# pachyderm-io/pfs

Hardware: AMD Instinct MI355X
Metric: GiB/s device-resident CDC rolling-hash + chunk content-hash (higher is better)
Workload: dtype u8

## Files before the change

### include/pfscdc.h

```cpp
#ifndef PFSCDC_H
#define PFSCDC_H

#include <stddef.h>
#include <stdint.h>

#ifdef __cplusplus
extern "C" {
#endif

#define PFSCDC_OK 0
#define PFSCDC_EINVAL -1
#define PFSCDC_EHIP -2
#define PFSCDC_ENOMEM -3
#define PFSCDC_EUNSUPPORTED -4
#define PFSCDC_ESTATE -5
#define PFSCDC_ECALLBACK -6
#define PFSCDC_ECORRUPT -7
#define PFSCDC_ENOTFOUND -8

typedef struct pfscdc_params {
  uint32_t average_bits;
  uint32_t reserved;
  int64_t seed;
  int64_t min_chunk;
// ... 43 lines not shown
int pfscdc_wait(pfscdc_ctx* ctx);

uint64_t pfscdc_num_segments(const pfscdc_ctx* ctx);
const pfscdc_segment* pfscdc_segments(const pfscdc_ctx* ctx);
const uint64_t* pfscdc_file_segment_begin(const pfscdc_ctx* ctx);

#define PFSCDC_OPT_REF_IDS 1u
#define PFSCDC_OPT_CUTS_ONLY 2u
#define PFSCDC_OPT_CTEXT_IN_PLACE 4u
int pfscdc_set_options(pfscdc_ctx* ctx, uint32_t options);
const pfscdc_ref* pfscdc_refs(const pfscdc_ctx* ctx);
int pfscdc_last_ref_ms(pfscdc_ctx* ctx, float* ms);

int pfscdc_get_chunks(pfscdc_ctx* ctx, const void* ctext, uint64_t nbytes, int ctext_on_device,
                      const uint64_t* chunk_offsets, uint32_t nchunks, const pfscdc_ref* refs,
                      void* ptext, int ptext_on_device, uint8_t* ok);
int pfscdc_last_get_ms(pfscdc_ctx* ctx, float* ms);

typedef struct pfscdc_slice {
  uint32_t chunk;
  uint32_t reserved;
  uint64_t offset;
  uint64_t size;
} pfscdc_slice;

int pfscdc_read_slices(pfscdc_ctx* ctx, const void* ctext, uint64_t nbytes, int ctext_on_device,
                       const uint64_t* chunk_offsets, uint32_t nchunks, const pfscdc_ref* refs,
                       const uint8_t* verified, const pfscdc_slice* slices, uint32_t nslices,
                       void* out, int out_on_device, uint8_t* chunk_ok, uint8_t* slice_ok);
int pfscdc_last_read_timings(pfscdc_ctx* ctx, float out[2]);

#define PFSCDC_TAR_USTAR 1
#define PFSCDC_TAR_PAX 2
typedef struct pfscdc_tar_file {
  const char* path;
  uint32_t first;
  uint32_t count;
} pfscdc_tar_file;

int pfscdc_tar_header(const char* path, uint64_t size, uint8_t out[512]);
int pfscdc_tar_layout(const pfscdc_tar_file* files, uint32_t nfiles, const uint64_t* sizes,
                      uint64_t* entry_offsets, uint64_t* total);
int pfscdc_tar_head(const char* path, uint64_t size, int format, uint8_t* out, uint64_t cap,
                    uint64_t* len);
int pfscdc_tar_layout_format(const pfscdc_tar_file* files, uint32_t nfiles, const uint64_t* sizes,
                             int format, uint64_t* entry_offsets, uint64_t* total);
int pfscdc_set_tar_format(pfscdc_ctx* ctx, int format);
int pfscdc_read_tar(pfscdc_ctx* ctx, const void* ctext, uint64_t nbytes, int ctext_on_device,
                    const uint64_t* chunk_offsets, uint32_t nchunks, const pfscdc_ref* refs,
                    const uint8_t* verified, const pfscdc_tar_file* files, uint32_t nfiles,
                    const pfscdc_slice* slices, uint32_t nslices, uint64_t begin, uint64_t len,
                    void* out, int out_on_device, uint8_t* chunk_ok, uint64_t* nwritten);
int pfscdc_last_frame_ms(pfscdc_ctx* ctx, float* ms);

int pfscdc_create_refs(pfscdc_ctx* ctx, const void* bytes, uint64_t nbytes, int bytes_on_device,
                       const uint64_t* chunk_offsets, uint32_t nchunks, uint8_t* content_hashes,
                       const uint8_t* hash_known, pfscdc_ref* refs);
int pfscdc_commit_refs(pfscdc_ctx* ctx, const void* bytes, uint64_t nbytes, int bytes_on_device,
                       const uint64_t* chunk_offsets, uint32_t nchunks, uint8_t* content_hashes,
                       const uint8_t* hash_known, pfscdc_ref* refs, uint8_t* segment_hashes);
int pfscdc_hash_data_refs(pfscdc_ctx* ctx, const uint8_t* hashes, uint32_t n, uint8_t out[32]);
int pfscdc_last_create_ms(pfscdc_ctx* ctx, float* ms);
int pfscdc_last_create_timings(pfscdc_ctx* ctx, float out[2]);
int pfscdc_last_create_form(pfscdc_ctx* ctx, int* split);


int pfscdc_candidates(pfscdc_ctx* ctx, const void* bytes, uint64_t nbytes, int bytes_on_device,
                      uint64_t halo, uint64_t* out, uint64_t cap, uint64_t* n);

int pfscdc_hash_ranges(pfscdc_ctx* ctx, const void* bytes, uint64_t nbytes, int bytes_on_device,
                       const uint64_t* begins, const uint64_t* sizes, uint32_t n, uint8_t* out);

uint64_t pfscdc_debug_candidates(pfscdc_ctx* ctx, uint64_t* out, uint64_t cap);

uint64_t pfscdc_debug_hash_queue(pfscdc_ctx* ctx, uint32_t* order, uint64_t order_cap,
                                 uint32_t* next, uint64_t next_cap, uint64_t* bin_bytes);
uint64_t pfscdc_debug_scan_plan(pfscdc_ctx* ctx, uint32_t* slots, uint64_t cap);

int pfscdc_last_scan_bytes(pfscdc_ctx* ctx, uint64_t* out);

int pfscdc_last_timings(pfscdc_ctx* ctx, float out[5]);
int pfscdc_last_kernel_spans(pfscdc_ctx* ctx, float out[2]);
int pfscdc_last_kernel_clocks(pfscdc_ctx* ctx, float out[2]);

void* pfscdc_host_alloc(uint64_t nbytes);
void pfscdc_host_free(void* p);

int pfscdc_fill_synthetic(pfscdc_ctx* ctx, void* dev_bytes, const uint64_t* file_offsets,
                          uint32_t nfiles, uint64_t seed);

#define PFSCDC_SYNTH_RANDOM 0u
#define PFSCDC_SYNTH_DEDUP_BLOCKS 1u
#define PFSCDC_SYNTH_DEDUP_FILES 2u
int pfscdc_fill_synthetic_ex(pfscdc_ctx* ctx, void* dev_bytes, const uint64_t* file_offsets,
                             uint32_t nfiles, uint64_t seed, uint32_t mode);
int pfscdc_fill_synthetic_pieces(pfscdc_ctx* ctx, void* dev_bytes, const uint64_t* piece_offsets,
                                 uint32_t npieces, const uint32_t* file_ids,
                                 const uint64_t* file_starts, uint64_t seed, uint32_t mode);


typedef struct pfscdc_dataref {
  uint8_t hash[32];
  int64_t offset_bytes;
  int64_t size_bytes;
} pfscdc_dataref;

typedef struct pfscdc_chunk_ref {
  uint64_t chunk_index;
  int64_t size_bytes;
  int32_t edge;
  int32_t has_ref;
  pfscdc_ref ref;
  int32_t copied;
  int32_t reserved2;
} pfscdc_chunk_ref;

typedef struct pfscdc_annotation_out {
  uint64_t user;
  int32_t has_data_ref;
  int32_t reserved;
  pfscdc_dataref data_ref;
} pfscdc_annotation_out;

typedef int (*pfscdc_writer_cb)(void* user, const pfscdc_chunk_ref* chunk,
                                const pfscdc_annotation_out* annotations, uint32_t n);

typedef struct pfscdc_writer pfscdc_writer;

typedef struct pfscdc_full_dataref {
  pfscdc_ref ref;
  int64_t ref_size;
  int32_t edge;
  int32_t reserved;
  pfscdc_dataref data;
} pfscdc_full_dataref;

typedef struct pfscdc_store pfscdc_store;
int pfscdc_store_create(pfscdc_store** out);
int pfscdc_store_destroy(pfscdc_store* s);
int pfscdc_store_put(pfscdc_store* s, const uint8_t id[32], const void* ctext, uint64_t n);
int pfscdc_store_get(const pfscdc_store* s, const uint8_t id[32], const void** ctext,
                     uint64_t* n);
uint64_t pfscdc_store_count(const pfscdc_store* s);
int pfscdc_store_read(pfscdc_ctx* ctx, const pfscdc_store* s, const pfscdc_full_dataref* drs,
                      uint32_t n, void* out, uint64_t out_cap, int out_on_device,
                      uint64_t* nwritten);
int pfscdc_store_read_tar(pfscdc_ctx* ctx, const pfscdc_store* s, const pfscdc_tar_file* files,
                          uint32_t nfiles, const pfscdc_full_dataref* drs, uint32_t ndrs,
                          uint64_t begin, uint64_t len, void* out, uint64_t out_cap,
                          int out_on_device, uint64_t* nwritten);

int pfscdc_writer_create(pfscdc_ctx* ctx, pfscdc_writer_cb cb, void* user,
                         uint64_t batch_bytes, pfscdc_writer** out);
int pfscdc_writer_annotate(pfscdc_writer* w, uint64_t user);
int pfscdc_writer_write(pfscdc_writer* w, const void* data, uint64_t n);
int pfscdc_writer_close(pfscdc_writer* w);
int64_t pfscdc_writer_chunk_count(const pfscdc_writer* w);
int64_t pfscdc_writer_annotation_count(const pfscdc_writer* w);
int pfscdc_writer_destroy(pfscdc_writer* w);

int pfscdc_writer_set_store(pfscdc_writer* w, pfscdc_store* store, int upload);
int pfscdc_writer_copy(pfscdc_writer* w, const pfscdc_full_dataref* dr);
int pfscdc_writer_prefetch(pfscdc_writer* w, const pfscdc_full_dataref* drs, uint32_t n);
int pfscdc_merge_file_hash(pfscdc_ctx* ctx, pfscdc_store* store, const pfscdc_full_dataref* drs,
                           uint32_t n, uint8_t out[32]);

// ... 267 lines not shown
```

### pfs_amd/_lib.py

```python
from __future__ import annotations

import ctypes as C
import os
import threading

_HERE = os.path.dirname(os.path.abspath(__file__))
LIB_PATH = os.environ.get("PFSCDC_LIB") or os.path.join(_HERE, "libpfscdc.so")

PFSCDC_OK = 0
PFSCDC_EINVAL = -1
PFSCDC_EHIP = -2
PFSCDC_ENOMEM = -3
PFSCDC_EUNSUPPORTED = -4
PFSCDC_ESTATE = -5
PFSCDC_ECALLBACK = -6
PFSCDC_ECORRUPT = -7
PFSCDC_ENOTFOUND = -8
TAR_USTAR, TAR_PAX = 1, 2

SEG_VALID = 1
SEG_CUT = 2
OPT_REF_IDS = 1
OPT_CUTS_ONLY = 2
OPT_CTEXT_IN_PLACE = 4
SCAN_SKIPPED_FIRST_MIN = 1
SCAN_SKIPPED_CUTS = 2

EXPORTED = [
    "pfscdc_default_params", "pfscdc_table", "pfscdc_go_int63", "pfscdc_ctx_create",
    "pfscdc_ctx_destroy", "pfscdc_last_error", "pfscdc_set_stream", "pfscdc_stream_wait",
    "pfscdc_stream_handle",
    "pfscdc_scan",
    "pfscdc_scan_async", "pfscdc_wait", "pfscdc_num_segments", "pfscdc_segments",
    "pfscdc_file_segment_begin", "pfscdc_debug_candidates", "pfscdc_debug_hash_queue",
    "pfscdc_debug_scan_plan", "pfscdc_last_timings",
    "pfscdc_last_scan_bytes", "pfscdc_commit_refs",
    "pfscdc_set_options", "pfscdc_refs", "pfscdc_last_ref_ms", "pfscdc_get_chunks",
    "pfscdc_last_get_ms",
    "pfscdc_host_alloc", "pfscdc_host_free", "pfscdc_fill_synthetic", "pfscdc_fill_synthetic_ex", "pfscdc_writer_create",
    "pfscdc_writer_annotate", "pfscdc_writer_write", "pfscdc_writer_close",
    "pfscdc_writer_chunk_count", "pfscdc_writer_annotation_count", "pfscdc_writer_destroy",
    "pfscdc_create_refs", "pfscdc_last_create_ms", "pfscdc_form_chunks",
    "pfscdc_uw_create", "pfscdc_uw_put", "pfscdc_uw_delete", "pfscdc_uw_close",
    "pfscdc_uw_num_filesets", "pfscdc_uw_fileset", "pfscdc_uw_destroy", "pfscdc_uw_last_error", "pfscdc_uw_timings",
    "pfscdc_uw_trim_cache", "pfscdc_uw_cached_arena_bytes",
    "pfscdc_path_clean",
    "pfscdc_hash_data_refs", "pfscdc_store_create", "pfscdc_store_destroy", "pfscdc_store_put",
    "pfscdc_store_get", "pfscdc_store_count", "pfscdc_writer_set_store", "pfscdc_writer_copy",
    "pfscdc_merge_file_hash", "pfscdc_last_create_timings", "pfscdc_last_create_form", "pfscdc_writer_prefetch",
    "pfscdc_candidates", "pfscdc_hash_ranges", "pfscdc_fill_synthetic_pieces",
    "pfscdc_last_kernel_spans", "pfscdc_last_kernel_clocks", "pfscdc_order_hash_after",
    "pfscdc_set_knob", "pfscdc_get_knob", "pfscdc_knob_info", "pfscdc_last_scan_mode",
    "pfscdc_deal", "pfscdc_group_create", "pfscdc_group_destroy", "pfscdc_group_size",
    "pfscdc_group_ctx", "pfscdc_group_last_error", "pfscdc_group_scan",
    "pfscdc_group_scan_resident", "pfscdc_group_num_segments", "pfscdc_group_segments",
    "pfscdc_group_file_segment_begin", "pfscdc_group_refs", "pfscdc_group_part_begin",
    "pfscdc_group_index_device", "pfscdc_group_last_timings", "pfscdc_uw_create_group",
    "pfscdc_group_scan_stream",
    "pfscdc_read_slices", "pfscdc_last_read_timings", "pfscdc_store_read",
    "pfscdc_tar_header", "pfscdc_tar_layout", "pfscdc_read_tar", "pfscdc_last_frame_ms",
    "pfscdc_store_read_tar", "pfscdc_tar_head", "pfscdc_tar_layout_format", "pfscdc_set_tar_format",
    "pfscdc_uw_set_store", "pfscdc_index_list_count", "pfscdc_index_list_entries",
    "pfscdc_index_list_blob", "pfscdc_index_list_datarefs", "pfscdc_index_list_tar_files",
    "pfscdc_index_list_free", "pfscdc_index_decode_host", "pfscdc_index_filter_list",
    "pfscdc_index_read", "pfscdc_last_index_stats", "pfscdc_last_index_timings",
    "pfscdc_index_merge", "pfscdc_index_merge_deletive", "pfscdc_index_merge_ctx",
    "pfscdc_last_merge_stats", "pfscdc_last_merge_timings", "pfscdc_shard",
    "pfscdc_fsw_create", "pfscdc_fsw_delete", "pfscdc_fsw_copy", "pfscdc_fsw_copy_lists",
    "pfscdc_fsw_copy_filesets", "pfscdc_fsw_close", "pfscdc_fsw_fileset",
    "pfscdc_fsw_last_error", "pfscdc_fsw_destroy",
    "pfscdc_dev_list_upload", "pfscdc_dev_list_download", "pfscdc_dev_list_count",
    "pfscdc_dev_list_num_datarefs", "pfscdc_dev_list_blob_len", "pfscdc_dev_list_free",
    "pfscdc_index_read_dev", "pfscdc_index_merge_dev", "pfscdc_dev_list_tar_layout",
    "pfscdc_dev_list_read_tar", "pfscdc_last_resident_stats",
    "pfscdc_source_host", "pfscdc_source_host_error", "pfscdc_file_infos_free",
    "pfscdc_source_open", "pfscdc_source_open_list", "pfscdc_source_list", "pfscdc_source_count",
    "pfscdc_source_infos", "pfscdc_source_free", "pfscdc_last_source_stats",
    "pfscdc_last_source_timings",
    "pfscdc_glob_match", "pfscdc_glob_literal_prefix", "pfscdc_debug_glob_program",
    "pfscdc_debug_glob_masks", "pfscdc_debug_list_scan",
    "pfscdc_diff_host", "pfscdc_diff_pairs_free", "pfscdc_source_diff", "pfscdc_diff_count",
    "pfscdc_diff_pairs", "pfscdc_diff_side", "pfscdc_diff_free", "pfscdc_last_diff_stats",
    "pfscdc_last_diff_timings",
    "pfscdc_copy_map_host", "pfscdc_dev_list_copy_map", "pfscdc_copy_map_list",
    "pfscdc_last_copy_map_stats", "pfscdc_last_copy_map_timings", "pfscdc_uw_copy",
    "pfscdc_uw_copy_file",
]


class Params(C.Structure):
    _fields_ = [("average_bits", C.c_uint32), ("reserved", C.c_uint32), ("seed", C.c_int64),
                ("min_chunk", C.c_int64), ("max_chunk", C.c_int64)]


class Segment(C.Structure):
    _fields_ = [("offset", C.c_uint64), ("size", C.c_uint64), ("file", C.c_uint32),
                ("flags", C.c_uint32), ("hash", C.c_uint8 * 32)]


class DataRef(C.Structure):
    _fields_ = [("hash", C.c_uint8 * 32), ("offset_bytes", C.c_int64), ("size_bytes", C.c_int64)]


class RefC(C.Structure):
    _fields_ = [("id", C.c_uint8 * 32), ("dek", C.c_uint8 * 32)]


class ChunkRef(C.Structure):
    _fields_ = [("chunk_index", C.c_uint64), ("size_bytes", C.c_int64), ("edge", C.c_int32),
                ("has_ref", C.c_int32), ("ref", RefC), ("copied", C.c_int32),
                ("reserved2", C.c_int32)]


class FullDataRef(C.Structure):
    _fields_ = [("ref", RefC), ("ref_size", C.c_int64), ("edge", C.c_int32),
                ("reserved", C.c_int32), ("data", DataRef)]


class TarFile(C.Structure):
    _fields_ = [("path", C.c_char_p), ("first", C.c_uint32), ("count", C.c_uint32)]


def tar_files(files):
    arr = (TarFile * max(1, len(files)))()
    for i, (path, first, count) in enumerate(files):
        p = path.encode() if isinstance(path, str) else bytes(path)
        if b"\0" in p:
            raise ValueError(f"tar entry {path!r}: NUL in the name")
        arr[i] = TarFile(p, first, count)
    return arr


class IndexFilter(C.Structure):
    _fields_ = [("lower", C.c_char_p), ("upper", C.c_char_p), ("prefix", C.c_char_p),
# ... 60 lines not shown


def slice_dtype():
    global SLICE_DTYPE
    if SLICE_DTYPE is None:
        import numpy as np
        SLICE_DTYPE = np.dtype([("chunk", "<u4"), ("reserved", "<u4"), ("offset", "<u8"),
                                ("size", "<u8")])
        assert SLICE_DTYPE.itemsize == 24
    return SLICE_DTYPE


def ref_dtype():
    global REF_DTYPE
    if REF_DTYPE is None:
        import numpy as np
        REF_DTYPE = np.dtype([("id", "u1", (32,)), ("dek", "u1", (32,))])
        assert REF_DTYPE.itemsize == 64
    return REF_DTYPE


def segment_dtype():
    global SEGMENT_DTYPE
    if SEGMENT_DTYPE is None:
        import numpy as np
        SEGMENT_DTYPE = np.dtype([("offset", "<u8"), ("size", "<u8"), ("file", "<u4"),
                                  ("flags", "<u4"), ("hash", "u1", (32,))])
        assert SEGMENT_DTYPE.itemsize == 56
    return SEGMENT_DTYPE


_lib = None
_lock = threading.Lock()


class PfsCdcError(RuntimeError):
    def __init__(self, code: int, msg: str):
        super().__init__(f"pfscdc error {code}: {msg}")
        self.code = code


def load() -> C.CDLL:
    global _lib
    with _lock:
        if _lib is not None:
            return _lib
        if not os.path.exists(LIB_PATH):
            raise ImportError(f"{LIB_PATH} is missing: build it with `make` or "
                              "`python -c 'import __graft_entry__ as g; g.build()'`")
        try:
            import torch
        except ImportError:
            pass
        lib = C.CDLL(LIB_PATH)
        u64, i64, u32, i32, vp = C.c_uint64, C.c_int64, C.c_uint32, C.c_int, C.c_void_p
        P = C.POINTER
        sig = {
            "pfscdc_default_params": (None, [P(Params)]),
            "pfscdc_table": (i32, [i64, P(u64)]),
            "pfscdc_go_int63": (i32, [i64, P(i64), i32]),
            "pfscdc_ctx_create": (i32, [P(Params), i32, P(vp)]),
            "pfscdc_ctx_destroy": (i32, [vp]),
            "pfscdc_last_error": (C.c_char_p, [vp]),
            "pfscdc_set_stream": (i32, [vp, vp]),
            "pfscdc_stream_wait": (i32, [vp, vp]),
            "pfscdc_stream_handle": (vp, [vp]),
            "pfscdc_order_hash_after": (i32, [vp, vp]),
            "pfscdc_scan": (i32, [vp, vp, u64, i32, P(u64), u32]),
            "pfscdc_scan_async": (i32, [vp, vp, u64, i32, P(u64), u32]),
            "pfscdc_wait": (i32, [vp]),
            "pfscdc_num_segments": (u64, [vp]),
            "pfscdc_segments": (P(Segment), [vp]),
            "pfscdc_file_segment_begin": (P(u64), [vp]),
            "pfscdc_debug_candidates": (u64, [vp, P(u64), u64]),
            "pfscdc_debug_hash_queue": (u64, [vp, vp, u64, vp, u64, P(u64)]),
            "pfscdc_debug_scan_plan": (u64, [vp, vp, u64]),
            "pfscdc_last_timings": (i32, [vp, P(C.c_float)]),
            "pfscdc_last_scan_bytes": (i32, [vp, P(u64)]),
            "pfscdc_last_scan_mode": (i32, [vp, P(u32)]),
            "pfscdc_set_knob": (i32, [C.c_char_p, i64]),
            "pfscdc_get_knob": (i32, [C.c_char_p, P(i64)]),
            "pfscdc_knob_info": (C.c_char_p, [i32, P(i64), P(i64), P(i64)]),
            "pfscdc_last_kernel_spans": (i32, [vp, P(C.c_float)]),
            "pfscdc_last_kernel_clocks": (i32, [vp, P(C.c_float)]),
            "pfscdc_set_options": (i32, [vp, u32]),
            "pfscdc_refs": (vp, [vp]),
            "pfscdc_last_ref_ms": (i32, [vp, P(C.c_float)]),
            "pfscdc_get_chunks": (i32, [vp, vp, u64, i32, P(u64), u32, vp, vp, i32, vp]),
            "pfscdc_last_get_ms": (i32, [vp, P(C.c_float)]),
            "pfscdc_host_alloc": (vp, [u64]),
            "pfscdc_host_free": (None, [vp]),
            "pfscdc_fill_synthetic": (i32, [vp, vp, P(u64), u32, u64]),
            "pfscdc_fill_synthetic_ex": (i32, [vp, vp, P(u64), u32, u64, u32]),
            "pfscdc_writer_create": (i32, [vp, WRITER_CB, vp, u64, P(vp)]),
            "pfscdc_writer_annotate": (i32, [vp, u64]),
            "pfscdc_writer_write": (i32, [vp, vp, u64]),
            "pfscdc_writer_close": (i32, [vp]),
            "pfscdc_writer_chunk_count": (i64, [vp]),
            "pfscdc_writer_annotation_count": (i64, [vp]),
            "pfscdc_writer_destroy": (i32, [vp]),
            "pfscdc_create_refs": (i32, [vp, vp, u64, i32, P(u64), u32, vp, vp, vp]),
            "pfscdc_commit_refs": (i32, [vp, vp, u64, i32, P(u64), u32, vp, vp, vp, vp]),
            "pfscdc_last_create_ms": (i32, [vp, P(C.c_float)]),
            "pfscdc_last_create_timings": (i32, [vp, P(C.c_float)]),
            "pfscdc_last_create_form": (i32, [vp, P(i32)]),
            "pfscdc_form_chunks": (i32, [vp, P(C.c_uint32), u32, P(u64), vp, vp, u64, P(u64)]),
            "pfscdc_uw_create": (i32, [vp, i64, P(Params), UW_CB, vp, P(vp)]),
            "pfscdc_uw_put": (i32, [vp, C.c_char_p, C.c_char_p, i32, vp, u64]),
            "pfscdc_uw_delete": (i32, [vp, C.c_char_p, C.c_char_p]),
            "pfscdc_uw_close": (i32, [vp]),
            "pfscdc_uw_num_filesets": (u32, [vp]),
            "pfscdc_uw_fileset": (i32, [vp, u32, P(FilesetInfo)]),
            "pfscdc_uw_destroy": (i32, [vp]),
            "pfscdc_uw_last_error": (C.c_char_p, [vp]),
            "pfscdc_uw_timings": (i32, [vp, P(C.c_double)]),
            "pfscdc_uw_trim_cache": (i32, [i32, P(u64), P(u32)]),
            "pfscdc_uw_cached_arena_bytes": (u64, []),
            "pfscdc_path_clean": (i32, [C.c_char_p, i32, C.c_char_p, u64]),
            "pfscdc_hash_data_refs": (i32, [vp, vp, u32, vp]),
            "pfscdc_store_create": (i32, [P(vp)]),
            "pfscdc_store_destroy": (i32, [vp]),
            "pfscdc_store_put": (i32, [vp, vp, vp, u64]),
            "pfscdc_store_get": (i32, [vp, vp, P(vp), P(u64)]),
            "pfscdc_store_count": (u64, [vp]),
            "pfscdc_writer_set_store": (i32, [vp, vp, i32]),
            "pfscdc_writer_copy": (i32, [vp, P(FullDataRef)]),
            "pfscdc_writer_prefetch": (i32, [vp, P(FullDataRef), u32]),
            "pfscdc_merge_file_hash": (i32, [vp, vp, P(FullDataRef), u32, vp]),
            "pfscdc_candidates": (i32, [vp, vp, u64, i32, u64, P(u64), u64, P(u64)]),
            "pfscdc_hash_ranges": (i32, [vp, vp, u64, i32, P(u64), P(u64), u32, vp]),
            "pfscdc_fill_synthetic_pieces": (i32, [vp, vp, P(u64), u32, P(C.c_uint32), P(u64),
                                                   u64, u32]),
            "pfscdc_deal": (i32, [P(u64), u32, u32, P(C.c_uint32)]),
            "pfscdc_group_create": (i32, [P(Params), P(C.c_int), u32, u32, P(vp)]),
            "pfscdc_group_destroy": (i32, [vp]),
            "pfscdc_group_size": (u32, [vp]),
            "pfscdc_group_ctx": (vp, [vp, u32]),
            "pfscdc_group_last_error": (C.c_char_p, [vp]),
            "pfscdc_group_scan": (i32, [vp, vp, u64, P(u64), u32]),
            "pfscdc_group_scan_resident": (i32, [vp, P(vp), P(u64), u32, P(C.c_uint32)]),
            "pfscdc_group_num_segments": (u64, [vp]),
            "pfscdc_group_segments": (vp, [vp]),
            "pfscdc_group_file_segment_begin": (P(u64), [vp]),
            "pfscdc_group_refs": (vp, [vp]),
            "pfscdc_group_part_begin": (P(C.c_uint32), [vp]),
            "pfscdc_group_index_device": (i32, [vp, P(vp), P(vp), P(C.c_int)]),
            "pfscdc_group_last_timings": (i32, [vp, P(C.c_float), P(C.c_float), P(u64)]),
            "pfscdc_uw_create_group": (i32, [vp, i64, P(Params), UW_CB, vp, P(vp)]),
            "pfscdc_group_scan_stream": (i32, [vp, vp, u64]),
            "pfscdc_read_slices": (i32, [vp, vp, u64, i32, P(u64), u32, vp, vp, vp, u32, vp, i32,
                                         vp, vp]),
            "pfscdc_last_read_timings": (i32, [vp, P(C.c_float)]),
            "pfscdc_store_read": (i32, [vp, vp, P(FullDataRef), u32, vp, u64, i32, P(u64)]),
            "pfscdc_tar_header": (i32, [C.c_char_p, u64, vp]),
            "pfscdc_tar_layout": (i32, [P(TarFile), u32, P(u64), P(u64), P(u64)]),
            "pfscdc_tar_head": (i32, [C.c_char_p, u64, i32, vp, u64, P(u64)]),
            "pfscdc_tar_layout_format": (i32, [P(TarFile), u32, P(u64), i32, P(u64), P(u64)]),
            "pfscdc_set_tar_format": (i32, [vp, i32]),
            "pfscdc_read_tar": (i32, [vp, vp, u64, i32, P(u64), u32, vp, vp, P(TarFile), u32, vp,
                                      u32, u64, u64, vp, i32, vp, P(u64)]),
            "pfscdc_last_frame_ms": (i32, [vp, P(C.c_float)]),
            "pfscdc_store_read_tar": (i32, [vp, vp, P(TarFile), u32, P(FullDataRef), u32, u64,
                                            u64, vp, u64, i32, P(u64)]),
            "pfscdc_uw_set_store": (i32, [vp, vp]),
            "pfscdc_index_list_count": (u32, [vp]),
            "pfscdc_index_list_entries": (P(IndexEntry), [vp]),
# ... 156 lines not shown
```

### pfs_amd/cdc.py

```python
from __future__ import annotations

import ctypes as C
from dataclasses import dataclass
from typing import Optional, Sequence

import numpy as np

from . import _lib


SYNTH_RANDOM, SYNTH_DEDUP_BLOCKS, SYNTH_DEDUP_FILES = 0, 1, 2


@dataclass(frozen=True)
class ChunkParams:
    average_bits: int = 23
    seed: int = 1
    min_chunk: int = 1_000_000
    max_chunk: int = 20_000_000

    def to_c(self) -> _lib.Params:
        return _lib.Params(self.average_bits, 0, self.seed, self.min_chunk, self.max_chunk)


# ... 63 lines not shown
            pass

    def _check(self, rc: int, what: str) -> None:
        if rc:
            msg = self.lib.pfscdc_last_error(self.ctx)
            raise _lib.PfsCdcError(rc, f"{what}: {msg.decode() if msg else ''}")

    def set_stream(self, stream_handle: Optional[int]) -> None:
        self._check(self.lib.pfscdc_set_stream(self.ctx, stream_handle or None), "set_stream")

    def order_hash_after(self, other: Optional["Chunker"]) -> None:
        self._check(self.lib.pfscdc_order_hash_after(self.ctx, other.ctx if other else None),
                    "order_hash_after")

    def wait_for(self, other: "Chunker") -> None:
        h = self.lib.pfscdc_stream_handle(other.ctx)
        self._check(self.lib.pfscdc_stream_wait(self.ctx, h), "stream_wait")

    def _after_torch(self, *tensors) -> None:
        for t in tensors:
            if t is not None and getattr(t, "is_cuda", False):
                import torch

                h = torch.cuda.current_stream(t.device).cuda_stream
                self._check(self.lib.pfscdc_stream_wait(self.ctx, h or None), "stream_wait")
                return

    def scan_async(self, data, file_offsets: Sequence[int]) -> None:
        offs = _offsets_array(file_offsets)
        self._offs_keep = offs
        nfiles = len(offs) - 1
        on_dev = 0
        if hasattr(data, "is_cuda") and data.is_cuda:
            if data.dtype.itemsize != 1 or not data.is_contiguous():
                raise ValueError("device data must be a contiguous uint8 tensor")
            ptr, nbytes, on_dev = data.data_ptr(), data.numel(), 1
            self._data_keep = data
            self._after_torch(data)
        else:
            arr = np.frombuffer(data, dtype=np.uint8) if isinstance(data, (bytes, bytearray, memoryview)) \
                else np.ascontiguousarray(data, dtype=np.uint8)
            self._data_keep = arr
            ptr, nbytes = (arr.ctypes.data if arr.size else None), arr.size
        rc = self.lib.pfscdc_scan_async(self.ctx, ptr, nbytes, on_dev,
                                        offs.ctypes.data_as(C.POINTER(C.c_uint64)), nfiles)
        self._check(rc, "scan_async")
        self._nfiles = nfiles

    def wait(self) -> ScanResult:
        self._check(self.lib.pfscdc_wait(self.ctx), "wait")
        n = self.lib.pfscdc_num_segments(self.ctx)
        dt = _lib.segment_dtype()
        if n:
            ptr = self.lib.pfscdc_segments(self.ctx)
            buf = C.string_at(ptr, n * dt.itemsize)
            segs = np.frombuffer(buf, dtype=dt).copy()
        else:
            segs = np.zeros(0, dtype=dt)
        bp = self.lib.pfscdc_file_segment_begin(self.ctx)
        begin = np.ctypeslib.as_array(bp, shape=(self._nfiles + 1,)).copy() if bp else \
            np.zeros(self._nfiles + 1, dtype=np.uint64)
        refs = None
        if self.ref_ids:
            rdt = _lib.ref_dtype()
            rp = self.lib.pfscdc_refs(self.ctx)
            refs = np.frombuffer(C.string_at(rp, n * rdt.itemsize), dtype=rdt).copy() \
                if (n and rp) else np.zeros(0, dtype=rdt)
        return ScanResult(segs, begin, refs=refs)

    def scan(self, data, file_offsets: Sequence[int]) -> ScanResult:
        self.scan_async(data, file_offsets)
        return self.wait()

    def timings(self) -> dict:
        out = (C.c_float * 5)()
        self._check(self.lib.pfscdc_last_timings(self.ctx, out), "timings")
        t = dict(zip(["scan", "compact", "select", "hash", "total"], list(out)))
        sp = (C.c_float * 2)()
        self._check(self.lib.pfscdc_last_kernel_spans(self.ctx, sp), "kernel_spans")
        t["scan_span"], t["hash_span"] = sp[0], sp[1]
        ck = (C.c_float * 2)()
        self._check(self.lib.pfscdc_last_kernel_clocks(self.ctx, ck), "kernel_clocks")
        t["scan_mhz"], t["hash_mhz"] = ck[0], ck[1]
        if self.ref_ids:
            ms = C.c_float()
            self._check(self.lib.pfscdc_last_ref_ms(self.ctx, C.byref(ms)), "timings")
            t["ref_ids"] = ms.value
        return t

    def get_chunks(self, ctext, chunk_offsets: Sequence[int], refs: np.ndarray, out=None):
        offs = _offsets_array(chunk_offsets)
        n = len(offs) - 1
        refs = np.ascontiguousarray(refs, dtype=_lib.ref_dtype())
        if len(refs) != n:
            raise ValueError("one ref per chunk")
        self._after_torch(ctext, out)
        if hasattr(ctext, "is_cuda") and ctext.is_cuda:
            cptr, nbytes, con = ctext.data_ptr(), ctext.numel(), 1
        else:
            arr = np.ascontiguousarray(np.frombuffer(ctext, dtype=np.uint8)
                                       if isinstance(ctext, (bytes, bytearray)) else ctext,
                                       dtype=np.uint8)
            cptr, nbytes, con = (arr.ctypes.data if arr.size else None), arr.size, 0
            self._get_keep = arr
        if out is not None:
            optr, oon, res = out.data_ptr(), 1, out
        else:
            res = np.empty(nbytes, dtype=np.uint8)
            optr, oon = (res.ctypes.data if nbytes else None), 0
        ok = np.zeros(max(n, 1), dtype=np.uint8)
        rc = self.lib.pfscdc_get_chunks(self.ctx, cptr, nbytes, con,
                                        offs.ctypes.data_as(C.POINTER(C.c_uint64)), n,
                                        refs.ctypes.data if n else None, optr, oon,
                                        ok.ctypes.data)
        self._check(rc, "get_chunks")
        return res, ok[:n].astype(bool)


    @staticmethod
    def _stored_batch(chunk_offsets, refs, slices, verified):
        offs = _offsets_array(chunk_offsets)
        n = len(offs) - 1
        refs = np.ascontiguousarray(refs, dtype=_lib.ref_dtype())
        if len(refs) != n:
            raise ValueError("one ref per chunk")
        sdt = _lib.slice_dtype()
        if isinstance(slices, np.ndarray) and slices.dtype == sdt:
            sl = np.ascontiguousarray(slices)
        else:
            sl = np.zeros(len(slices), dtype=sdt)
            for i, (ch, o, z) in enumerate(slices):
                sl[i] = (ch, 0, o, z)
        ver = None
        if verified is not None:
            ver = np.ascontiguousarray(np.asarray(verified).astype(np.uint8))
            if len(ver) != n:
                raise ValueError("one verified mark per chunk")
        return offs, n, refs, sl, len(sl), ver

    def _ctext_arg(self, ctext):
        if hasattr(ctext, "is_cuda") and ctext.is_cuda:
            if ctext.dtype.itemsize != 1 or not ctext.is_contiguous():
                raise ValueError("device ctext must be a contiguous uint8 tensor")
            return ctext.data_ptr(), ctext.numel(), 1
        arr = np.ascontiguousarray(np.frombuffer(ctext, dtype=np.uint8)
                                   if isinstance(ctext, (bytes, bytearray)) else ctext,
                                   dtype=np.uint8)
        self._get_keep = arr
        return (arr.ctypes.data if arr.size else None), arr.size, 0

    @staticmethod
    def _out_arg(out, need: int, what: str):
        if out is None:
            res = np.empty(need, dtype=np.uint8)
            return res, (res.ctypes.data if need else None), 0
        if isinstance(out, np.ndarray):
            if out.dtype != np.uint8 or not out.flags.c_contiguous or out.size < need:
                raise ValueError(f"out must be a contiguous uint8 array of {what}")
            return out, (out.ctypes.data if out.size else None), 0
        if out.dtype.itemsize != 1 or not out.is_contiguous() or out.numel() < need:
            raise ValueError(f"out must be a contiguous uint8 tensor of {what}")
        return out, (out.data_ptr() if out.numel() else None), int(out.is_cuda)

    def read_slices(self, ctext, chunk_offsets: Sequence[int], refs: np.ndarray, slices,
                    out=None, verified=None):
        offs, n, refs, sl, ns, ver = self._stored_batch(chunk_offsets, refs, slices, verified)
# ... 317 lines not shown
```

### pfs_amd/csrc/cdc_kernels.hip

```cpp
#include <hip/hip_runtime.h>
#include <stdint.h>
#include <stdlib.h>

#include <algorithm>
#include <type_traits>

#include "pfscdc_internal.h"

#define PFS_DEV __device__ __forceinline__

namespace pfscdc {


PFS_DEV uint64_t rotl1_64(uint64_t x) { return (x << 1) | (x >> 63); }

PFS_DEV uint32_t tab_addr(uint32_t w, uint32_t lane_off, int j) {
  return __builtin_amdgcn_perm(w, lane_off, 0x0c0c0000u | ((4u + (uint32_t)j) << 8));
}

template <typename T>
PFS_DEV T lds_load(const uint8_t* lds, uint32_t byte_addr) {
  return *reinterpret_cast<const T*>(lds + byte_addr);
}

// ... 589 lines not shown
  __syncthreads();
  if (threadIdx.x == 0) {
    __threadfence();
    *s_flag = atomicAdd(done_ctr, 1u) == gridDim.x - 1 ? 1u : 0u;
  }
  __syncthreads();
  const bool last = *s_flag != 0;
  if (last) __threadfence();
  return last;
}

template <int BLOCK>
PFS_DEV void compact_tiles(const TileRec* __restrict__ recs, uint64_t ntiles, uint64_t n,
                           uint64_t* __restrict__ entries, uint64_t* __restrict__ n_entries,
                           uint64_t* s_wave) {
  uint64_t carry = 0;
  for (uint64_t base = 0; base < ntiles; base += BLOCK) {
    const uint64_t t = base + threadIdx.x;
    uint32_t c = 0;
    uint64_t e = 0;
    if (t < ntiles) {
      c = recs[t].count;
      e = c <= (uint32_t)kTileK ? c : 1;
    }
    uint64_t total;
    const uint64_t ex = block_exscan<BLOCK>(e, s_wave, &total) + carry;
    if (t < ntiles) {
      const uint64_t ts = t * kTile;
      if (c <= (uint32_t)kTileK) {
        uint32_t o[kTileK];
#pragma unroll
        for (int i = 0; i < kTileK; i++) o[i] = i < (int)c ? recs[t].off[i] : ~0u;
#pragma unroll
        for (int i = 0; i < kTileK; i++) {
          uint32_t rank = 0;
#pragma unroll
          for (int j = 0; j < kTileK; j++) rank += o[j] < o[i];
          if (i < (int)c) entries[ex + rank] = ts + o[i];
        }
      } else {
        const uint64_t te = (ts + kTile < n) ? ts + kTile : n;
        entries[ex] = kDenseBit | (te - 1);
      }
    }
    carry += total;
  }
  if (threadIdx.x == 0) *n_entries = carry;
}

template <int BLOCK>
PFS_DEV uint64_t segcompact_block(const pfscdc_segment* __restrict__ slots,
                                  const uint64_t* __restrict__ seg_base,
                                  const uint64_t* __restrict__ nseg, uint32_t nfiles,
                                  pfscdc_segment* __restrict__ segs,
                                  uint64_t* __restrict__ seg_begin, uint64_t* s_wave) {
  uint64_t carry = 0;
  for (uint64_t base = 0; base < nfiles; base += BLOCK) {
    const uint64_t f = base + threadIdx.x;
    const uint64_t c = f < nfiles ? nseg[f] : 0;
    uint64_t total;
    const uint64_t ex = block_exscan<BLOCK>(c, s_wave, &total) + carry;
    if (f < nfiles) {
      seg_begin[f] = ex;
      const pfscdc_segment* src = slots + seg_base[f];
      for (uint64_t i = 0; i < c; i++) segs[ex + i] = src[i];
    }
    carry += total;
  }
  if (threadIdx.x == 0) seg_begin[nfiles] = carry;
  return carry;
}

PFS_DEV uint32_t lpt_key(uint64_t size) {
  const uint64_t nblk = (size + 127) / 128;
  const uint64_t k = nblk >> 6;
  return 1023u - (uint32_t)(k < 1023 ? k : 1023);
}

template <int BLOCK>
PFS_DEV void lpt_order_block(const pfscdc_segment* __restrict__ segs, uint64_t n,
                             uint32_t* __restrict__ order, uint32_t* __restrict__ counter,
                             uint32_t* hist, uint64_t* s_wave,
                             const uint64_t* __restrict__ offs = nullptr, uint64_t bin_bytes = 0,
                             uint32_t* __restrict__ next = nullptr, uint64_t* qlen = nullptr) {
  const bool bins = next && offs && bin_bytes;
  auto binned = [&](uint64_t i) {
    const uint32_t f = segs[i].file;
    return bins && offs[f + 1] - offs[f] <= bin_bytes;
  };
  auto entry = [&](uint64_t i, uint32_t& key) {
    if (binned(i)) {
      const uint32_t f = segs[i].file;
      key = lpt_key(offs[f + 1] - offs[f]);
      return i == 0 || segs[i - 1].file != f;
    }
    key = lpt_key(segs[i].size);
    return true;
  };
  constexpr int kPer = 1024 / BLOCK;
  static_assert(1024 % BLOCK == 0, "bins split evenly over the block");
  for (int b = 0; b < kPer; b++) hist[threadIdx.x * kPer + b] = 0;
  __syncthreads();
  for (uint64_t i = threadIdx.x; i < n; i += BLOCK) {
    uint32_t key;
    if (entry(i, key)) atomicAdd(&hist[key], 1u);
    if (bins) next[i] = binned(i) && i + 1 < n && segs[i + 1].file == segs[i].file
                            ? (uint32_t)(i + 1) : kNoNext;
  }
  __syncthreads();
  uint32_t local[kPer];
  uint64_t sum = 0;
  for (int b = 0; b < kPer; b++) {
    local[b] = hist[threadIdx.x * kPer + b];
    sum += local[b];
  }
  uint64_t total;
  uint64_t start = block_exscan<BLOCK>(sum, s_wave, &total);
  for (int b = 0; b < kPer; b++) {
    hist[threadIdx.x * kPer + b] = (uint32_t)start;
    start += local[b];
  }
  __syncthreads();
  for (uint64_t i = threadIdx.x; i < n; i += BLOCK) {
    uint32_t key;
    if (entry(i, key)) order[atomicAdd(&hist[key], 1u)] = (uint32_t)i;
  }
  if (threadIdx.x == 0) {
    *counter = 0;
    if (qlen) *qlen = total;
  }
}


PFS_DEV uint64_t rescan_first(const uint8_t* __restrict__ data, const uint64_t* __restrict__ T,
                              uint64_t a, uint64_t b, uint64_t mask) {
  const uint32_t lane = threadIdx.x & 63u;
  constexpr uint64_t W = 256;
  for (uint64_t base = a; base <= b; base += 64 * W) {
    const uint64_t st = base + lane * W;
    const uint64_t en = (st + W - 1 < b) ? st + W - 1 : b;
    uint64_t found = kNone;
    if (st <= en) {
      uint64_t h = 0;
      for (int k = 0; k < 64; k++) h = rotl1_64(h) ^ T[data[st - 63 + k]];
      if ((h & mask) == 0) found = st;
      for (uint64_t i = st + 1; found == kNone && i <= en; i++) {
        h = rotl1_64(h) ^ T[data[i - 64]] ^ T[data[i]];
        if ((h & mask) == 0) found = i;
      }
    }
    found = wave_min_u64(found);
    if (found != kNone) return found;
  }
  return kNone;
}

PFS_DEV void select_file(
    const uint8_t* __restrict__ data, const uint64_t* __restrict__ T,
    const uint64_t* __restrict__ entries, const uint64_t* __restrict__ n_entries,
    const uint64_t* __restrict__ offs, const uint64_t* __restrict__ seg_base, uint64_t f,
    uint64_t mask, uint64_t min_chunk, uint64_t max_chunk,
    pfscdc_segment* __restrict__ slots, uint64_t* __restrict__ nseg) {
  const uint32_t lane = threadIdx.x & 63u;
  const uint64_t fs = offs[f], fe = offs[f + 1];
  const uint64_t sb = seg_base[f], cap = seg_base[f + 1] - sb;
  const uint64_t ne = *n_entries;
  pfscdc_segment* out = slots + sb;
  uint64_t count = 0;
  auto emit = [&](uint64_t s, uint64_t size, uint32_t flags) {
    if (lane == 0 && count < cap) {
      out[count].offset = s - fs;
      out[count].size = size;
      out[count].file = (uint32_t)f;
      out[count].flags = flags;
    }
    count++;
  };
  uint64_t k = 0;
  {
    const uint64_t key = fs + min_chunk - 1;
    uint64_t lo = 0, hi = ne;
    while (hi - lo > 64) {
      const uint64_t step = (hi - lo + 63) / 64;
      const uint64_t i = lo + lane * step;
      const bool below = i < hi && (entries[i] & ~kDenseBit) < key;
      const uint32_t cnt = (uint32_t)__popcll(__ballot(below));
      if (cnt == 0) {
        hi = lo;
      } else {
        const uint64_t top = lo + (uint64_t)cnt * step;
        lo = lo + (uint64_t)(cnt - 1) * step + 1;
        hi = top < hi ? top : hi;
      }
    }
    const uint64_t i = lo + lane;
    const bool below = i < hi && (entries[i] & ~kDenseBit) < key;
    k = lo + (uint64_t)__popcll(__ballot(below));
  }
  uint64_t s = fs;
  while (true) {
    const uint64_t lo = s + min_chunk - 1;
    if (lo >= fe) break;
    const uint64_t hi = s + max_chunk - 1;
    const uint64_t limit = hi < fe - 1 ? hi : fe - 1;
    while (k < ne && (entries[k] & ~kDenseBit) < lo) k++;
    uint64_t c = kNone;
    for (uint64_t kk = k; kk < ne; kk++) {
      const uint64_t e = entries[kk];
      const uint64_t v = e & ~kDenseBit;
      if (!(e & kDenseBit)) {
        if (v <= limit) c = v;
        break;
      }
      const uint64_t ts = (v / kTile) * kTile;
      const uint64_t a = lo > ts ? lo : ts;
      const uint64_t bnd = v < limit ? v : limit;
      if (a <= bnd) {
        c = rescan_first(data, T, a, bnd, mask);
        if (c != kNone) break;
      }
      if (v >= limit) break;
    }
    uint64_t cut;
    if (c != kNone) cut = c;
    else if (hi <= fe - 1) cut = hi;
    else break;
    emit(s, cut + 1 - s, PFSCDC_SEG_VALID | PFSCDC_SEG_CUT);
    s = cut + 1;
  }
  if (s < fe) emit(s, fe - s, PFSCDC_SEG_VALID);
  if (lane == 0) {
    for (uint64_t i = count; i < cap; i++) out[i].flags = 0;
    nseg[f] = count;
  }
}

__global__ __launch_bounds__(kSelectBlock) void select_kernel(
    const uint8_t* __restrict__ data, const uint64_t* __restrict__ T,
    const uint64_t* __restrict__ entries, const uint64_t* __restrict__ n_entries,
    const uint64_t* __restrict__ offs, const uint64_t* __restrict__ seg_base, uint32_t nfiles,
    uint64_t mask, uint64_t min_chunk, uint64_t max_chunk,
    pfscdc_segment* __restrict__ slots, uint64_t* __restrict__ nseg, uint32_t* done_ctr,
    pfscdc_segment* __restrict__ segs, uint64_t* __restrict__ seg_begin,
    uint32_t* __restrict__ order, uint32_t* __restrict__ counter, uint64_t bin_bytes,
    uint32_t* __restrict__ next, uint64_t* __restrict__ qlen) {
  __shared__ uint32_t hist[1024];
  __shared__ uint64_t s_wave[kSelectBlock / 64 + 1];
  __shared__ uint32_t s_flag;
  const uint64_t f = ((uint64_t)blockIdx.x * kSelectBlock + threadIdx.x) >> 6;
  if (f < nfiles)
    select_file(data, T, entries, n_entries, offs, seg_base, f, mask, min_chunk, max_chunk,
                slots, nseg);
  if (!last_block_done(done_ctr, &s_flag)) return;
  const uint64_t total = segcompact_block<kSelectBlock>(slots, seg_base, nseg, nfiles, segs,
                                                        seg_begin, s_wave);
  __threadfence_block();
  __syncthreads();
  if (order)
    lpt_order_block<kSelectBlock>(segs, total, order, counter, hist, s_wave, offs, bin_bytes,
                                  next, qlen);
}


__global__ __launch_bounds__(kCompactBlock) void hash_order_kernel(
    const pfscdc_segment* __restrict__ segs, const uint64_t* __restrict__ seg_count,
    uint32_t* __restrict__ order, uint32_t* __restrict__ counter) {
  __shared__ uint32_t hist[1024];
  __shared__ uint64_t s_wave[kCompactBlock / 64 + 1];
  lpt_order_block<kCompactBlock>(segs, *seg_count, order, counter, hist, s_wave);
}


constexpr uint64_t kB2IV[8] = {
    0x6a09e667f3bcc908ULL, 0xbb67ae8584caa73bULL, 0x3c6ef372fe94f82bULL,
    0xa54ff53a5f1d36f1ULL, 0x510e527fade682d1ULL, 0x9b05688c2b3e6c1fULL,
    0x1f83d9abfb41bd6bULL, 0x5be0cd19137e2179ULL};

template <typename T>
PFS_DEV T pick4(uint32_t j, T v0, T v1, T v2, T v3) {
  return j == 0 ? v0 : j == 1 ? v1 : j == 2 ? v2 : v3;
}

constexpr uint32_t kSigmaPack[12][4] = {
#define PK(a, b, c, d) ((uint32_t)(a) * 8u | (uint32_t)(b) * 8u << 8 | (uint32_t)(c) * 8u << 16 | (uint32_t)(d) * 8u << 24)
#define ROW(s0, s1, s2, s3, s4, s5, s6, s7, s8, s9, s10, s11, s12, s13, s14, s15) \
  {PK(s0, s1, s14, s15), PK(s2, s3, s8, s9), PK(s4, s5, s10, s11), PK(s6, s7, s12, s13)}
    ROW(0, 1, 2, 3, 4, 5, 6, 7, 8, 9, 10, 11, 12, 13, 14, 15),
    ROW(14, 10, 4, 8, 9, 15, 13, 6, 1, 12, 0, 2, 11, 7, 5, 3),
    ROW(11, 8, 12, 0, 5, 2, 15, 13, 10, 14, 3, 6, 7, 1, 9, 4),
    ROW(7, 9, 3, 1, 13, 12, 11, 14, 2, 6, 5, 10, 4, 0, 15, 8),
    ROW(9, 0, 5, 7, 2, 4, 10, 15, 14, 1, 11, 12, 6, 8, 3, 13),
    ROW(2, 12, 6, 10, 0, 11, 8, 3, 4, 13, 7, 5, 15, 14, 1, 9),
    ROW(12, 5, 1, 15, 14, 13, 4, 10, 0, 7, 6, 3, 9, 2, 8, 11),
    ROW(13, 11, 7, 14, 12, 1, 3, 9, 5, 0, 15, 4, 8, 6, 2, 10),
    ROW(6, 15, 14, 9, 11, 3, 0, 8, 12, 2, 13, 7, 1, 4, 10, 5),
    ROW(10, 2, 8, 4, 7, 6, 1, 5, 15, 11, 9, 14, 3, 12, 13, 0),
    ROW(0, 1, 2, 3, 4, 5, 6, 7, 8, 9, 10, 11, 12, 13, 14, 15),
    ROW(14, 10, 4, 8, 9, 15, 13, 6, 1, 12, 0, 2, 11, 7, 5, 3),
#undef ROW
#undef PK
};

PFS_DEV uint64_t mk64(uint32_t lo, uint32_t hi) { return ((uint64_t)hi << 32) | lo; }
PFS_DEV uint64_t xor_rotr32(uint64_t x, uint64_t y) {
  return mk64((uint32_t)(x >> 32) ^ (uint32_t)(y >> 32), (uint32_t)x ^ (uint32_t)y);
}
template <int N>
PFS_DEV uint64_t xor_rotr(uint64_t x, uint64_t y) {
  const uint32_t lo = (uint32_t)x ^ (uint32_t)y, hi = (uint32_t)(x >> 32) ^ (uint32_t)(y >> 32);
  return mk64(__builtin_amdgcn_alignbit(hi, lo, N), __builtin_amdgcn_alignbit(lo, hi, N));
}
PFS_DEV uint64_t xor_rotr63(uint64_t x, uint64_t y) {
  const uint32_t lo = (uint32_t)x ^ (uint32_t)y, hi = (uint32_t)(x >> 32) ^ (uint32_t)(y >> 32);
  return mk64(__builtin_amdgcn_alignbit(lo, hi, 31), __builtin_amdgcn_alignbit(hi, lo, 31));
}

template <int CTRL>
PFS_DEV uint64_t quad_perm64(uint64_t x) {
  const uint32_t lo = (uint32_t)__builtin_amdgcn_mov_dpp((int)(uint32_t)x, CTRL, 0xF, 0xF, true);
  const uint32_t hi = (uint32_t)__builtin_amdgcn_mov_dpp((int)(uint32_t)(x >> 32), CTRL, 0xF, 0xF, true);
  return mk64(lo, hi);
}

#define PFS_G(a, b, c, d, x, y)  \
  do {                           \
    a = a + b + (x);             \
    d = xor_rotr32(d, a);        \
    c = c + d;                   \
    b = xor_rotr<24>(b, c);      \
    a = a + b + (y);             \
    d = xor_rotr<16>(d, a);      \
    c = c + d;                   \
    b = xor_rotr63(b, c);        \
  } while (0)

PFS_DEV void msg_load_full(uint4& m0, uint4& m1, const uint8_t* p) {
  __builtin_memcpy(&m0, p, 16);
  __builtin_memcpy(&m1, p + 16, 16);
}

PFS_DEV uint32_t keep_bytes(int64_t k) {
  return k >= 4 ? 0xffffffffu : k <= 0 ? 0u : (1u << (8 * (uint32_t)k)) - 1u;
}
// ... 136 lines not shown
  "v_lshl_add_u64 v[100:101], v[100:101], 0, v[102:103]\n"             \
  "v_xor_b32 v110, v108, v100\n"                                       \
  "v_xor_b32 v111, v109, v101\n"                                       \
  "v_alignbit_b32 v106, v111, v110, 16\n"                              \
  "v_alignbit_b32 v107, v110, v111, 16\n"                              \
  "v_lshl_add_u64 v[104:105], v[104:105], 0, v[106:107]\n"             \
  "v_xor_b32 v110, v102, v104\n"                                       \
  "v_xor_b32 v111, v103, v105\n"                                       \
  "v_alignbit_b32 v102, v110, v111, 31\n"                              \
  "v_alignbit_b32 v103, v111, v110, 31\n"
#define PFS_G_ASM_FIRST(X, Y)                                          \
  "v_lshl_add_u64 v[100:101], %[a0], 0, " X "\n"                      \
  "v_lshl_add_u64 v[100:101], v[100:101], 0, %[b0]\n"                 \
  "v_bitop3_b32 v108, %[d0h], %[dth], v101 bitop3:0x96\n"             \
  "v_bitop3_b32 v109, %[d0l], %[dtl], v100 bitop3:0x96\n"             \
  "v_lshl_add_u64 v[104:105], %[c0], 0, v[108:109]\n"                 \
  "v_xor_b32 v110, %[b0l], v104\n"                                    \
  "v_xor_b32 v111, %[b0h], v105\n"                                    \
  "v_alignbit_b32 v102, v111, v110, 24\n"                             \
  "v_alignbit_b32 v103, v110, v111, 24\n"                             \
  "v_lshl_add_u64 v[100:101], v[100:101], 0, " Y "\n"                 \
  "v_lshl_add_u64 v[100:101], v[100:101], 0, v[102:103]\n"            \
  "v_xor_b32 v110, v108, v100\n"                                      \
  "v_xor_b32 v111, v109, v101\n"                                      \
  "v_alignbit_b32 v106, v111, v110, 16\n"                             \
  "v_alignbit_b32 v107, v110, v111, 16\n"                             \
  "v_lshl_add_u64 v[104:105], v[104:105], 0, v[106:107]\n"            \
  "v_xor_b32 v110, v102, v104\n"                                      \
  "v_xor_b32 v111, v103, v105\n"                                      \
  "v_alignbit_b32 v102, v110, v111, 31\n"                             \
  "v_alignbit_b32 v103, v111, v110, 31\n"
#define PFS_QP_ID "[0,1,2,3]"
#define PFS_QP_R1 "[1,2,3,0]"
#define PFS_QP_R2 "[2,3,0,1]"
#define PFS_QP_R3 "[3,0,1,2]"
#define PFS_DIAG_G PFS_G_ASM(PFS_QP_R3, PFS_QP_R1, PFS_QP_R2, "%[x2l]", "%[x2h]", "%[x3]")
#define PFS_ROUND_OPS(x0_, x1_, x2_, x3_)                                                \
  : "+{v[100:101]}"(a), "+{v[102:103]}"(b), "+{v[104:105]}"(c), "+{v[106:107]}"(d)      \
  : [x0] "v"(x0_), [x0l] "v"((uint32_t)(x0_)), [x0h] "v"((uint32_t)((x0_) >> 32)),      \
    [x1] "v"(x1_), [x2l] "v"((uint32_t)(x2_)), [x2h] "v"((uint32_t)((x2_) >> 32)),       \
    [x3] "v"(x3_)                                                                        \
  : "vcc", "v108", "v109", "v110", "v111"
#define PFS_ROUND_FIRST(a0_, b0_, c0_, d0_, dt_, x0_, x1_, x2_, x3_)                          \
  asm volatile(PFS_G_ASM_FIRST("%[x0]", "%[x1]") PFS_DIAG_G                                    \
               : "=&{v[100:101]}"(a), "=&{v[102:103]}"(b), "=&{v[104:105]}"(c),                  \
                 "=&{v[106:107]}"(d)                                                           \
               : [a0] "v"(a0_), [b0] "v"(b0_), [b0l] "v"((uint32_t)(b0_)),                     \
                 [b0h] "v"((uint32_t)((b0_) >> 32)), [c0] "v"(c0_),                            \
                 [d0l] "v"((uint32_t)(d0_)), [d0h] "v"((uint32_t)((d0_) >> 32)),               \
                 [dtl] "v"((uint32_t)(dt_)), [dth] "v"((uint32_t)((dt_) >> 32)),               \
                 [x0] "v"(x0_), [x1] "v"(x1_), [x2l] "v"((uint32_t)(x2_)),                      \
                 [x2h] "v"((uint32_t)((x2_) >> 32)), [x3] "v"(x3_)                              \
               : "vcc", "v108", "v109", "v110", "v111")
#define PFS_ROUND(FIRST, x0_, x1_, x2_, x3_)                                                  \
  do {                                                                                        \
    if (FIRST)                                                                                \
      asm volatile(PFS_G_ASM_PLAIN("%[x0]", "%[x1]") PFS_DIAG_G                    \
                 PFS_ROUND_OPS(x0_, x1_, x2_, x3_));                                          \
    else                                                                                      \
      asm volatile(PFS_G_ASM(PFS_QP_R1, PFS_QP_R3, PFS_QP_R2, "%[x0l]", "%[x0h]", \
                                         "%[x1]") PFS_DIAG_G                                   \
                 PFS_ROUND_OPS(x0_, x1_, x2_, x3_));                                          \
  } while (0)

PFS_DEV void fold_diag(uint64_t& ha, uint64_t& hb, uint64_t a, uint64_t b, uint64_t c, uint64_t d) {
  uint32_t hal = (uint32_t)ha, hah = (uint32_t)(ha >> 32), hbl = (uint32_t)hb,
           hbh = (uint32_t)(hb >> 32);
  asm volatile(
      "v_xor_b32_dpp %0, %4, %0 quad_perm:[1,2,3,0] row_mask:0xf bank_mask:0xf\n"
      "v_xor_b32_dpp %1, %5, %1 quad_perm:[1,2,3,0] row_mask:0xf bank_mask:0xf\n"
      "v_xor_b32_dpp %0, %6, %0 quad_perm:[3,0,1,2] row_mask:0xf bank_mask:0xf\n"
      "v_xor_b32_dpp %1, %7, %1 quad_perm:[3,0,1,2] row_mask:0xf bank_mask:0xf\n"
      "v_xor_b32 %2, %8, %2\n"
      "v_xor_b32 %3, %9, %3\n"
      "v_xor_b32_dpp %2, %10, %2 quad_perm:[2,3,0,1] row_mask:0xf bank_mask:0xf\n"
      "v_xor_b32_dpp %3, %11, %3 quad_perm:[2,3,0,1] row_mask:0xf bank_mask:0xf\n"
      : "+v"(hal), "+v"(hah), "+v"(hbl), "+v"(hbh)
      : "v"((uint32_t)a), "v"((uint32_t)(a >> 32)), "v"((uint32_t)c), "v"((uint32_t)(c >> 32)),
        "v"((uint32_t)b), "v"((uint32_t)(b >> 32)), "v"((uint32_t)d), "v"((uint32_t)(d >> 32)));
  ha = ((uint64_t)hah << 32) | hal;
  hb = ((uint64_t)hbh << 32) | hbl;
}

constexpr int kModeHash = 0, kModeRefId = 1, kModeGet = 2;
template <int MODE>
__global__ __launch_bounds__(kHashBlock) __attribute__((amdgpu_waves_per_eu(1, 2))) void blake2b_kernel(
    const uint8_t* __restrict__ data, const uint64_t* __restrict__ offs,
    pfscdc_segment* __restrict__ segs, const uint64_t* __restrict__ seg_count,
    const uint32_t* __restrict__ order, uint32_t* __restrict__ counter, uint64_t nbytes,
    pfscdc_ref* __restrict__ refs, uint8_t* __restrict__ out, uint32_t prio_blocks,
    uint64_t* span, const uint32_t* __restrict__ next, uint64_t* __restrict__ fair,
    uint32_t fair_every) {
  constexpr bool CIPHER = MODE != kModeHash;
  const SpanClock span_clk = span_begin(span);
  constexpr uint32_t kMsgStride = 160, kMsgBuf = kHashBlock / 4 * kMsgStride;
  __shared__ __attribute__((aligned(16))) uint8_t s_msg[2 * kMsgBuf];
  const uint8_t* const end = data + nbytes;
  const uint32_t lane = threadIdx.x & 63u;
  const uint32_t j = lane & 3u;
  const uint64_t nseg = *seg_count;
  const uint32_t slot = (threadIdx.x >> 2) * kMsgStride;
  uint8_t* my = s_msg + slot + 32u * j;

  const uint32_t lds_base = (uint32_t)(uintptr_t)(const __attribute__((address_space(3))) uint8_t*)s_msg;
  uint32_t ma[10][4];
#pragma unroll
  for (int r = 0; r < 10; r++) {
    const uint32_t pk = pick4(j, kSigmaPack[r][0], kSigmaPack[r][1], kSigmaPack[r][2], kSigmaPack[r][3]);
#pragma unroll
    for (int k = 0; k < 4; k++) {
      ma[r][k] = lds_base + slot + ((pk >> (8 * k)) & 0xFFu);
      asm volatile("" : "+v"(ma[r][k]));
    }
  }
  const uint64_t iv_c = pick4(j, kB2IV[0], kB2IV[1], kB2IV[2], kB2IV[3]);
  const uint64_t iv_d = pick4(j, kB2IV[4], kB2IV[5], kB2IV[6], kB2IV[7]);
  const uint64_t h0a = j == 0 ? (kB2IV[0] ^ 0x01010020ULL) : iv_c;
  const uint64_t t_mask = j == 0 ? ~0ULL : 0ULL;
  const uint64_t h0b = iv_d;

  if (prio_blocks == kHashPrioAuto)
    prio_blocks = nseg > (uint64_t)gridDim.x * (kHashBlock / 4) ? 8192u : 0u;
  bool active = false;
  uint32_t bin_next = kNoNext;
  bool drained = false;
  uint32_t quiet = 0;
  uint64_t L = 0, nblk = 0, blk = 0;
  const uint8_t* src = data;
  pfscdc_segment* seg = segs;
  uint32_t sidx = 0;
  uint64_t ha = 0, hb = 0;
  uint4 m0 = make_uint4(0, 0, 0, 0), m1 = m0;
  uint32_t key_b = 0, key_c = 0;
  uint8_t* dst_base = out;
  const uint32_t cc_a = pick4(j, 0x61707865u, 0x3320646eu, 0x79622d32u, 0x6b206574u);

  auto lds_put = [&](uint32_t buf) {
    reinterpret_cast<uint4*>(my + buf)[0] = m0;
    reinterpret_cast<uint4*>(my + buf)[1] = m1;
  };
  auto load_block = [&](uint64_t b) {
    const uint8_t* p = src + b * 128 + 32 * j;
    if (b + 1 == nblk) msg_load_tail(m0, m1, p, (int64_t)(L - b * 128) - 32 * (int64_t)j, end);
    else msg_load_full(m0, m1, p);
  };

  auto store_block = [&](uint32_t buf) {
    const int64_t avail = (int64_t)(L - blk * 128) - 32 * (int64_t)j;
    if (active && avail > 0) {
      const uint4 p0 = reinterpret_cast<const uint4*>(my + buf)[0];
      const uint4 p1 = reinterpret_cast<const uint4*>(my + buf)[1];
      uint8_t* o = dst_base + blk * 128 + 32 * j;
      if (avail >= 32) {
        __builtin_memcpy(o, &p0, 16);
        __builtin_memcpy(o + 16, &p1, 16);
      } else {
        uint8_t tmp[32];
        __builtin_memcpy(tmp, &p0, 16);
        __builtin_memcpy(tmp + 16, &p1, 16);
        for (int64_t k = 0; k < avail; k++) o[k] = tmp[k];
      }
    }
  };

  auto rounds = [&](auto par, uint64_t& a, uint64_t& b, uint64_t& c, uint64_t& d,
                    auto&& put_next, uint64_t* pre = nullptr, bool back = true,
                    uint64_t dt = 0) {
    constexpr uint32_t cur = decltype(par)::value * kMsgBuf, nxt = kMsgBuf - cur;
    __builtin_amdgcn_fence(__ATOMIC_RELEASE, "wavefront");
    __builtin_amdgcn_wave_barrier();
    __builtin_amdgcn_fence(__ATOMIC_ACQUIRE, "wavefront");
    uint64_t x0, x1, x2, x3;
    if (pre) {
      x0 = pre[0]; x1 = pre[1]; x2 = pre[2]; x3 = pre[3];
    } else {
      x0 = lds_abs_u64(ma[0][0] + cur); x1 = lds_abs_u64(ma[0][1] + cur);
      x2 = lds_abs_u64(ma[0][2] + cur); x3 = lds_abs_u64(ma[0][3] + cur);
    }
    uint64_t sv[2][4];
#pragma unroll
    for (int r = 0; r < 12; r++) {
      if (r < 2) {
        sv[r][0] = x0; sv[r][1] = x1; sv[r][2] = x2; sv[r][3] = x3;
      }
      uint64_t y0 = 0, y1 = 0, y2 = 0, y3 = 0;
      if (r == 9 || r == 10) {
        y0 = sv[r - 9][0]; y1 = sv[r - 9][1]; y2 = sv[r - 9][2]; y3 = sv[r - 9][3];
      } else if (r < 11) {
        y0 = lds_abs_u64(ma[r + 1][0] + cur);
        y1 = lds_abs_u64(ma[r + 1][1] + cur);
        y2 = lds_abs_u64(ma[r + 1][2] + cur);
        y3 = lds_abs_u64(ma[r + 1][3] + cur);
      } else if (pre) {
        __builtin_amdgcn_fence(__ATOMIC_RELEASE, "wavefront");
        __builtin_amdgcn_wave_barrier();
        __builtin_amdgcn_fence(__ATOMIC_ACQUIRE, "wavefront");
        pre[0] = lds_abs_u64(ma[0][0] + nxt);
        pre[1] = lds_abs_u64(ma[0][1] + nxt);
        pre[2] = lds_abs_u64(ma[0][2] + nxt);
        pre[3] = lds_abs_u64(ma[0][3] + nxt);
      }
      if (r == 0) {
        const uint64_t a0 = a, b0 = b, c0 = c, d0 = d;
        PFS_ROUND_FIRST(a0, b0, c0, d0, dt, x0, x1, x2, x3);
      } else {
        PFS_ROUND(false, x0, x1, x2, x3);
      }
      x0 = y0; x1 = y1; x2 = y2; x3 = y3;
      if (r == 5) put_next();
    }
    if (back) {
      a = quad_perm64<0x39>(a);
      c = quad_perm64<0x93>(c);
      d = quad_perm64<0x4E>(d);
    }
  };

  const uint32_t kFairEvery = fair_every ? fair_every : 256;
  uint32_t wave_steps = 0;
  uint32_t reported = 0;
  const uint64_t nwaves = (uint64_t)gridDim.x * (kHashBlock / 64);
  uint64_t tm = 0;
  const uint64_t tinc = 128 & t_mask;
  auto fast_step = [&](auto par, uint64_t* pre) {
    constexpr uint32_t cur = decltype(par)::value * kMsgBuf, nxt = kMsgBuf - cur;
    uint64_t a = ha, b = hb, c = iv_c, d = iv_d;
    rounds(par, a, b, c, d, [&] {
      if (active) {
        lds_put(nxt);
        msg_load_full(m0, m1, src + (blk + 2) * 128 + 32 * j);
      }
    }, pre, false, tm);
    fold_diag(ha, hb, a, b, c, d);
    tm += tinc;
    blk++;
  };

  auto step = [&](auto par) -> bool {
    constexpr uint32_t cur = decltype(par)::value * kMsgBuf, nxt = kMsgBuf - cur;
    bool fast = false;
    if (quiet) {
      quiet--;
      fast = quiet >= 3;
    } else {
      auto begin = [&](uint32_t s) {
        sidx = s;
        seg = segs + sidx;
        L = seg->size;
        if (CIPHER) {
          const uint32_t* dk = reinterpret_cast<const uint32_t*>(refs[sidx].dek);
          key_b = dk[j];
          key_c = dk[4 + j];
        }
        src = data + offs[seg->file] + seg->offset;
        if (MODE != kModeHash && out) dst_base = out + offs[seg->file] + seg->offset;
        nblk = L == 0 ? 1 : (L + 127) / 128;
        blk = 0;
        ha = h0a;
        hb = h0b;
        active = true;
        load_block(0);
        lds_put(cur);
        if (nblk > 1) load_block(1);
      };
      if (!active && bin_next != kNoNext) {
        begin(bin_next);
        bin_next = kNoNext;
      }
      if (!drained) {
        const bool need = !active;
        const uint64_t want = __ballot(need && j == 0);
        if (want) {
          const uint32_t cnt = (uint32_t)__popcll(want);
          const uint32_t leader = (uint32_t)__builtin_ctzll(want);
          uint32_t base = 0;
          if (lane == leader) base = atomicAdd(counter, cnt);
          base = (uint32_t)__shfl((int)base, (int)leader, 64);
          if (need) {
            const uint64_t below = want & ((1ULL << (lane & ~3u)) - 1);
            const uint64_t idx = (uint64_t)base + (uint64_t)__popcll(below);
            if (idx < nseg) begin(order[idx]);
          }
          if ((uint64_t)base + cnt >= nseg) drained = true;
        }
      }
      if (__ballot(active) == 0) return false;
      if (fair) {
        const uint32_t d = wave_steps - reported;
        uint64_t tot = 0;
        if (lane == 0) tot = atomicAdd((unsigned long long*)fair, (unsigned long long)d);
        tot = ((uint64_t)__builtin_amdgcn_readfirstlane((uint32_t)(tot >> 32)) << 32) |
              (uint32_t)__builtin_amdgcn_readfirstlane((uint32_t)tot);
        reported = wave_steps;
        const uint64_t mine = (uint64_t)wave_steps * nwaves, all = tot + d;
        if (mine < all) __builtin_amdgcn_s_setprio(1);
        else __builtin_amdgcn_s_setprio(0);
      } else if (prio_blocks) {
        const uint64_t T = prio_blocks, rem = active ? nblk - blk : 0;
        if (__ballot(rem > T)) __builtin_amdgcn_s_setprio(2);
        else __builtin_amdgcn_s_setprio(0);
      }

      const uint64_t rem64 = active ? nblk - blk : 0;
      const uint32_t rem = rem64 > 0xffffffffULL ? 0xffffffffu : (uint32_t)rem64;
      uint32_t q = wave_min_u32(active ? rem : 0xffffffffu) - 1;
      if (fair && q > kFairEvery - 1) q = kFairEvery - 1;
      if (!fair && prio_blocks) {
        const uint32_t T = prio_blocks, rmax = wave_max_u32(rem);
        if (rmax > T && rmax - T - 1 < q) q = rmax - T - 1;
      }
      quiet = q;
    }
    const bool last = !fast && blk + 1 == nblk;
    if (MODE == kModeRefId) {
      __builtin_amdgcn_fence(__ATOMIC_RELEASE, "wavefront");
      __builtin_amdgcn_wave_barrier();
      __builtin_amdgcn_fence(__ATOMIC_ACQUIRE, "wavefront");
      const int64_t avail = (int64_t)(L - blk * 128);
#pragma unroll
      for (int h = 0; h < 2; h++) {
        uint32_t ks[4];
        chacha20_column(ks, cc_a, key_b, key_c, j == 0 ? (uint32_t)(2 * blk + h) : 0u);
        uint32_t* dst = reinterpret_cast<uint32_t*>(s_msg + cur + slot + 64 * h) + j;
#pragma unroll
        for (int w = 0; w < 4; w++) {
          const uint32_t v = last ? ks[w] & keep_bytes(avail - 64 * h - 16 * w - 4 * (int64_t)j) : ks[w];
          __hip_atomic_fetch_xor(dst + 4 * w, v, __ATOMIC_RELAXED, __HIP_MEMORY_SCOPE_WORKGROUP);
        }
      }
      if (out) {
        __builtin_amdgcn_fence(__ATOMIC_RELEASE, "wavefront");
        __builtin_amdgcn_wave_barrier();
        __builtin_amdgcn_fence(__ATOMIC_ACQUIRE, "wavefront");
        store_block(cur);
      }
    }
    uint64_t a = ha, b = hb, c = iv_c, d;
    if (fast) {
      d = iv_d ^ (((blk + 1) << 7) & t_mask);
    } else {
      const uint64_t t = last ? L : (blk + 1) * 128;
      d = iv_d ^ (j == 0 ? t : 0) ^ ((j == 2 && last) ? ~0ULL : 0);
    }
    rounds(par, a, b, c, d, [&] {
      if (active && !last) {
        lds_put(nxt);
        if (blk + 2 < nblk) load_block(blk + 2);
      }
    });
    ha ^= a ^ c;
    hb ^= b ^ d;
    if (MODE == kModeGet) {
      __builtin_amdgcn_fence(__ATOMIC_RELEASE, "wavefront");
      __builtin_amdgcn_wave_barrier();
      __builtin_amdgcn_fence(__ATOMIC_ACQUIRE, "wavefront");
#pragma unroll
      for (int h = 0; h < 2; h++) {
        uint32_t ks[4];
        chacha20_column(ks, cc_a, key_b, key_c, j == 0 ? (uint32_t)(2 * blk + h) : 0u);
        uint32_t* dst = reinterpret_cast<uint32_t*>(s_msg + cur + slot + 64 * h) + j;
#pragma unroll
        for (int w = 0; w < 4; w++)
          __hip_atomic_fetch_xor(dst + 4 * w, ks[w], __ATOMIC_RELAXED, __HIP_MEMORY_SCOPE_WORKGROUP);
      }
      __builtin_amdgcn_fence(__ATOMIC_RELEASE, "wavefront");
      __builtin_amdgcn_wave_barrier();
      __builtin_amdgcn_fence(__ATOMIC_ACQUIRE, "wavefront");
      store_block(cur);
    }
    if (fast) {
      blk++;
    } else if (active) {
      blk++;
      if (last) {
        if (MODE == kModeRefId) reinterpret_cast<uint64_t*>(refs[sidx].id)[j] = ha;
        else reinterpret_cast<uint64_t*>(seg->hash)[j] = ha;
        active = false;
        if (next) bin_next = next[sidx];
      }
    }
    return true;
  };
  constexpr std::integral_constant<uint32_t, 0> P0{};
  constexpr std::integral_constant<uint32_t, 1> P1{};
  while (true) {
    if (!step(P0)) break;
    if (!step(P1)) break;
    wave_steps += 2;
    if constexpr (MODE == kModeHash) {
      if (quiet >= 5) {
        uint64_t pre[4] = {lds_abs_u64(ma[0][0]), lds_abs_u64(ma[0][1]), lds_abs_u64(ma[0][2]),
                           lds_abs_u64(ma[0][3])};
        tm = ((blk + 1) << 7) & t_mask;
        do {
          fast_step(P0, pre);
          fast_step(P1, pre);
          quiet -= 2;
          wave_steps += 2;
        } while (quiet >= 5);
      }
    }
  }
  span_end(span, span_clk);
}

PFS_DEV uint32_t rotl32v(uint32_t x, int n) { return __builtin_amdgcn_alignbit(x, x, 32 - n); }
#define PFS_CQR(a, b, c, d)                         \
  do {                                              \
    x[a] += x[b]; x[d] = rotl32v(x[d] ^ x[a], 16);  \
    x[c] += x[d]; x[b] = rotl32v(x[b] ^ x[c], 12);  \
    x[a] += x[b]; x[d] = rotl32v(x[d] ^ x[a], 8);   \
    x[c] += x[d]; x[b] = rotl32v(x[b] ^ x[c], 7);   \
  } while (0)
constexpr int kChachaBlock = 256;
__global__ __launch_bounds__(kChachaBlock) void chacha_xor_coalesced_kernel(
    const uint8_t* data, const uint64_t* __restrict__ offs,
    const pfscdc_segment* __restrict__ segs, const uint64_t* __restrict__ blk_base, uint32_t n,
    const pfscdc_ref* __restrict__ refs, uint8_t* out, uint32_t prio) {
  if (prio) __builtin_amdgcn_s_setprio(2);
  __shared__ __attribute__((aligned(16))) uint32_t s_ks[kChachaBlock / 64][64 * 16];
  __shared__ uint64_t s_at[kChachaBlock / 64][64];
  __shared__ int64_t s_avail[kChachaBlock / 64][64];
  const uint64_t nblocks = blk_base[n];
  const uint64_t stride = (uint64_t)gridDim.x * blockDim.x;
  const uint32_t lane = threadIdx.x & 63u;
  const uint32_t wv = threadIdx.x >> 6;
  uint32_t* const ks = s_ks[wv];
  const uint64_t w0 = (uint64_t)blockIdx.x * blockDim.x +
                      (uint32_t)__builtin_amdgcn_readfirstlane((int)(threadIdx.x & ~63u));
  for (uint64_t g0 = w0; g0 < nblocks; g0 += stride) {
    uint32_t lo = 0, hi = n;
    while (hi - lo > 1) {
      const uint32_t mid = (lo + hi) >> 1;
      if (blk_base[mid] <= g0) lo = mid;
      else hi = mid;
    }
    const uint64_t g = g0 + lane;
    uint32_t x[16];
    uint64_t at = 0;
    int64_t avail = 0;
    if (g < nblocks) {
      while (blk_base[lo + 1] <= g) lo++;
      const pfscdc_segment& sg = segs[lo];
      const uint64_t b = g - blk_base[lo];
      at = offs[sg.file] + sg.offset + 64 * b;
      avail = (int64_t)(sg.size - 64 * b);
      const uint4 k0 = reinterpret_cast<const uint4*>(refs[lo].dek)[0];
      const uint4 k1 = reinterpret_cast<const uint4*>(refs[lo].dek)[1];
      const uint32_t s[16] = {0x61707865u, 0x3320646eu, 0x79622d32u, 0x6b206574u,
                              k0.x, k0.y, k0.z, k0.w, k1.x, k1.y, k1.z, k1.w,
                              (uint32_t)b, 0u, 0u, 0u};
#pragma unroll
      for (int i = 0; i < 16; i++) x[i] = s[i];
#pragma unroll
      for (int r = 0; r < 10; r++) {
        PFS_CQR(0, 4, 8, 12);
        PFS_CQR(1, 5, 9, 13);
        PFS_CQR(2, 6, 10, 14);
        PFS_CQR(3, 7, 11, 15);
        PFS_CQR(0, 5, 10, 15);
        PFS_CQR(1, 6, 11, 12);
        PFS_CQR(2, 7, 8, 13);
        PFS_CQR(3, 4, 9, 14);
      }
#pragma unroll
      for (int i = 0; i < 16; i++) x[i] += s[i];
    } else {
#pragma unroll
      for (int i = 0; i < 16; i++) x[i] = 0;
    }
    __builtin_amdgcn_wave_barrier();
#pragma unroll
    for (int q = 0; q < 4; q++) {
      const uint32_t slot = ((uint32_t)q + (lane >> 1)) & 3u;
      *reinterpret_cast<uint4*>(ks + lane * 16 + 4 * slot) =
          make_uint4(x[4 * q], x[4 * q + 1], x[4 * q + 2], x[4 * q + 3]);
    }
    s_at[wv][lane] = at;
    s_avail[wv][lane] = avail;
    __builtin_amdgcn_fence(__ATOMIC_RELEASE, "wavefront");
    __builtin_amdgcn_wave_barrier();
    __builtin_amdgcn_fence(__ATOMIC_ACQUIRE, "wavefront");
// ... 451 lines not shown
      const uint32_t mid = (lo + hi) >> 1;
      if (offs[mid] <= g) lo = mid;
      else hi = mid;
    }
    uint32_t f = lo;
    uint8_t bytes[8];
    for (int b = 0; b < 8; b++) {
      const uint64_t p = g + b;
      if (p >= n) break;
      while (f + 1 < nfiles && offs[f + 1] <= p) f++;
      const uint64_t o = p - offs[f] + (starts ? starts[f] : 0);
      const uint64_t fid = ids ? ids[f] : f;
      bytes[b] = (uint8_t)(synth_byte_word(fid, o, seed, mode) >> (8 * (o & 7)));
    }
    if (g + 8 <= n) {
      uint64_t w;
      __builtin_memcpy(&w, bytes, 8);
      *reinterpret_cast<uint64_t*>(out + g) = w;
    } else {
      for (uint64_t p = g; p < n; p++) out[p] = bytes[p - g];
    }
  }
}


hipError_t prepare_kernels() {
  const int lds = (int)kScanLdsBytes;
  hipError_t e = hipFuncSetAttribute((const void*)cdc_scan_kernel<false>,
                                     hipFuncAttributeMaxDynamicSharedMemorySize, lds);
  if (e != hipSuccess) return e;
  return hipFuncSetAttribute((const void*)cdc_scan_kernel<true>,
                             hipFuncAttributeMaxDynamicSharedMemorySize, lds);
}

hipError_t launch_scan_skip(const uint64_t* offs, uint32_t nfiles, uint64_t n, uint64_t min_chunk,
                            uint64_t ntiles, uint32_t* skip, uint64_t* scanned, hipStream_t st) {
  const uint64_t nunits = ntiles * kScanWaves;
  if (nunits == 0) return hipSuccess;
  scan_skip_kernel<<<(unsigned)((nunits + 255) / 256), 256, 0, st>>>(
      offs, nfiles, n, min_chunk, nunits, skip, (unsigned long long*)scanned, nullptr, nullptr);
  return hipGetLastError();
}

hipError_t launch_scan_plan(const uint64_t* offs, uint32_t nfiles, uint64_t n, uint64_t min_chunk,
                            uint64_t ntiles, uint32_t* skip, uint64_t* scanned, uint32_t* uinfo,
                            uint4* slots, uint32_t* plan, const ScanPlan& hdr, ScanPlan* d_hdr,
                            hipStream_t st) {
  const uint64_t nunits = ntiles * kScanWaves;
  if (nunits == 0) return hipSuccess;
  const unsigned grid = (unsigned)((nunits + 255) / 256);
  scan_skip_kernel<<<grid, 256, 0, st>>>(offs, nfiles, n, min_chunk, nunits, skip,
                                         (unsigned long long*)scanned, uinfo, plan);
  hipError_t e = hipGetLastError();
  if (e != hipSuccess) return e;
  scan_slots_kernel<<<grid, 256, 0, st>>>(nunits, uinfo, plan, slots, hdr, d_hdr);
  return hipGetLastError();
}

hipError_t launch_scan(const uint8_t* data, const uint8_t* tail, uint64_t n, const uint64_t* d_table,
                       uint32_t average_bits, uint64_t ntiles, TileRec* recs, int grid,
                       uint32_t* unit_ctr, uint32_t* done_ctr, uint64_t* entries,
                       uint64_t* n_entries, uint64_t* span, hipStream_t st, const uint32_t* skip,
                       const ScanPlan* d_plan) {
  const size_t lds = kScanLdsBytes;
  const uint64_t mask64 = average_bits >= 64 ? ~0ULL : ((1ULL << average_bits) - 1);
  const ScanPlan* const pl = d_plan;
  if (average_bits <= 32)
    cdc_scan_kernel<false><<<grid, kScanBlock, lds, st>>>(
        data, tail, n, d_table, 32 - average_bits, mask64, ntiles, recs, unit_ctr, done_ctr,
        entries, n_entries, skip, span, pl);
  else
    cdc_scan_kernel<true><<<grid, kScanBlock, lds, st>>>(
        data, tail, n, d_table, 64 - average_bits, mask64, ntiles, recs, unit_ctr, done_ctr,
        entries, n_entries, skip, span, pl);
  return hipGetLastError();
}

hipError_t launch_select(const uint8_t* data, const uint64_t* d_table, const uint64_t* entries,
                         const uint64_t* n_entries, const uint64_t* offs,
                         const uint64_t* seg_base, uint32_t nfiles, uint32_t average_bits,
                         uint64_t min_chunk, uint64_t max_chunk, pfscdc_segment* slots,
                         uint64_t* nseg, uint32_t* done_ctr, pfscdc_segment* segs,
                         uint64_t* seg_begin, uint32_t* order, uint32_t* counter,
                         hipStream_t st, uint64_t bin_bytes, uint32_t* next, uint64_t* qlen) {
  const uint64_t mask64 = average_bits >= 64 ? ~0ULL : ((1ULL << average_bits) - 1);
  const uint64_t waves_per_block = kSelectBlock / 64;
  const uint64_t grid = (nfiles + waves_per_block - 1) / waves_per_block;
  select_kernel<<<(unsigned)grid, kSelectBlock, 0, st>>>(data, d_table, entries, n_entries,
                                                         offs, seg_base, nfiles, mask64,
                                                         min_chunk, max_chunk, slots, nseg,
                                                         done_ctr, segs, seg_begin, order,
                                                         counter, bin_bytes, next, qlen);
  return hipGetLastError();
}

static uint32_t prio_arg(uint32_t prio) {
  return prio == kHashPrioNone ? 0u : prio ? prio : kHashPrioAuto;
}

int hash_waves(uint64_t longest_bytes, uint64_t total_bytes, int num_cus, int forced) {
  if (forced >= 1 && forced <= 8) return forced;
  const uint64_t quads1 = (uint64_t)num_cus * 4 * (64 / 4);
  const uint64_t longest = (longest_bytes + 127) / 128, total = total_bytes / 128;
  return longest * quads1 >= total ? 1 : kHashWavesPerSimd;
}

static unsigned hash_grid(uint64_t max_segments, int num_cus, int waves) {
  const uint64_t quads_per_block = kHashBlock / 4;
  const uint64_t need = (max_segments + quads_per_block - 1) / quads_per_block;
  const uint64_t full = (uint64_t)num_cus * 4 * (waves > 0 ? waves : kHashWavesPerSimd) /
                        (kHashBlock / 64);
  return capped_grid(need < full ? need : full, Knob::HashGrid);
}

hipError_t launch_blake2b(const uint8_t* data, const uint64_t* offs, pfscdc_segment* segs,
                          const uint64_t* seg_count, uint64_t max_segments, uint32_t* order,
                          uint32_t* counter, int num_cus, uint64_t nbytes, hipStream_t st,
                          bool ordered, uint64_t* span, int waves, uint32_t prio,
                          bool cu_exclusive, const uint32_t* next, uint64_t* fair,
                          uint32_t fair_every) {
  if (max_segments == 0) return hipSuccess;
  if (!ordered) hash_order_kernel<<<1, kCompactBlock, 0, st>>>(segs, seg_count, order, counter);
  const size_t dyn = cu_exclusive ? 64u * 1024u : 0u;
  blake2b_kernel<kModeHash><<<hash_grid(max_segments, num_cus, waves), kHashBlock, dyn, st>>>(
      data, offs, segs, seg_count, order, counter, nbytes, nullptr, nullptr,
      prio_arg(prio), span, ordered ? next : nullptr, ordered ? fair : nullptr, fair_every);
  return hipGetLastError();
}

hipError_t launch_order(const pfscdc_segment* segs, const uint64_t* seg_count, uint32_t* order,
                        uint32_t* counter, hipStream_t st) {
  hash_order_kernel<<<1, kCompactBlock, 0, st>>>(segs, seg_count, order, counter);
  return hipGetLastError();
}

hipError_t launch_ref_ids(const uint8_t* data, const uint64_t* offs, pfscdc_segment* segs,
                          const uint64_t* seg_count, uint64_t max_segments, const uint32_t* order,
                          uint32_t* counter, int num_cus, uint64_t nbytes, pfscdc_ref* refs,
                          uint8_t* ctext_out, hipStream_t st, int waves, uint32_t prio,
                          const uint32_t* next, const uint64_t* nsegs) {
  if (max_segments == 0) return hipSuccess;
  dek_kernel<<<(unsigned)((max_segments + 255) / 256), 256, 0, st>>>(
      segs, nsegs ? nsegs : seg_count, refs, counter);
  blake2b_kernel<kModeRefId><<<hash_grid(max_segments, num_cus, waves), kHashBlock, 0, st>>>(
      data, offs, segs, seg_count, order, counter, nbytes, refs, ctext_out,
      prio_arg(prio), nullptr, next, nullptr, 0u);
  return hipGetLastError();
}

hipError_t launch_deks(pfscdc_segment* segs, const uint64_t* seg_count, uint64_t max_segments,
                       pfscdc_ref* refs, uint32_t* counter, hipStream_t st) {
  if (max_segments == 0) return hipSuccess;
  dek_kernel<<<(unsigned)((max_segments + 255) / 256), 256, 0, st>>>(segs, seg_count, refs, counter);
  return hipGetLastError();
}

hipError_t launch_chacha_xor(const uint8_t* data, const uint64_t* offs, const pfscdc_segment* segs,
                             const uint64_t* blk_base, uint32_t n, uint64_t nblocks,
                             const pfscdc_ref* refs, uint8_t* out, int num_cus, hipStream_t st,
                             bool prio, bool one_wave_per_simd) {
  if (nblocks == 0) return hipSuccess;
  const uint64_t need = (nblocks + 255) / 256,
                 full = (uint64_t)num_cus * (one_wave_per_simd ? 1 : 32);
  const unsigned grid = capped_grid(need < full ? need : full, Knob::ChachaGrid);
  chacha_xor_coalesced_kernel<<<grid, kChachaBlock, 0, st>>>(data, offs, segs, blk_base, n,
                                                            refs, out, prio ? 1u : 0u);
  return hipGetLastError();
}

hipError_t launch_get(const uint8_t* ctext, const uint64_t* offs, pfscdc_segment* segs,
                      const uint64_t* seg_count, uint64_t nsegs, uint32_t* order, uint32_t* counter,
                      int num_cus, uint64_t nbytes, pfscdc_ref* refs, uint8_t* ptext, hipStream_t st,
                      int waves) {
  if (nsegs == 0) return hipSuccess;
  hash_order_kernel<<<1, kCompactBlock, 0, st>>>(segs, seg_count, order, counter);
  blake2b_kernel<kModeGet><<<hash_grid(nsegs, num_cus, waves), kHashBlock, 0, st>>>(
      ctext, offs, segs, seg_count, order, counter, nbytes, refs, ptext, prio_arg(0), nullptr,
      nullptr, nullptr, 0u);
  return hipGetLastError();
}

hipError_t launch_verify_ids(const pfscdc_segment* segs, uint32_t n, const pfscdc_ref* refs,
                             uint8_t* ok, hipStream_t st) {
  if (n == 0) return hipSuccess;
  verify_ids_kernel<<<(n + 255) / 256, 256, 0, st>>>(segs, n, refs, ok);
  return hipGetLastError();
}

hipError_t launch_slice_gather(const uint8_t* ctext, const uint64_t* chunk_offs,
                               const pfscdc_ref* refs, const uint8_t* ok,
                               const pfscdc_slice* slices, const uint64_t* out_off,
                               const uint64_t* blk_base, uint32_t n, uint64_t nblocks,
                               uint8_t* out, int num_cus, hipStream_t st) {
  if (nblocks == 0) return hipSuccess;
  const uint64_t need = (nblocks + kChachaBlock - 1) / kChachaBlock, full = (uint64_t)num_cus * 32;
  chacha_slice_gather_kernel<<<capped_grid(need < full ? need : full, Knob::ChachaGrid),
                               kChachaBlock, 0, st>>>(
      ctext, chunk_offs, refs, ok, slices, out_off, blk_base, n, out);
  return hipGetLastError();
}

hipError_t launch_tar_frame(const TarEntry* d_entries, const uint8_t* d_names, uint32_t n,
                            const uint64_t* d_xblk, uint64_t nx, uint64_t begin, uint64_t end,
                            uint64_t total, uint8_t* out, int num_cus, hipStream_t st) {
  if (end <= begin) return hipSuccess;
  if (!d_xblk) nx = 0;
  const uint64_t per = kTarBlock / 64, need = ((uint64_t)n + 2 + nx + per - 1) / per,
                 full = (uint64_t)num_cus * 8;
  const unsigned grid = capped_grid(need < full ? need : full, Knob::ChachaGrid);
  if (nx)
    tar_frame_kernel<true><<<grid, kTarBlock, 0, st>>>(d_entries, d_names, n, d_xblk, nx, begin,
                                                       end, total, out);
  else
    tar_frame_kernel<false><<<grid, kTarBlock, 0, st>>>(d_entries, d_names, n, nullptr, 0, begin,
                                                        end, total, out);
  return hipGetLastError();
}

hipError_t launch_synth(uint8_t* out, const uint64_t* offs, uint32_t nfiles, const uint32_t* ids,
                        const uint64_t* starts, uint64_t seed, uint32_t mode, hipStream_t st) {
  synth_kernel<<<2048, 256, 0, st>>>(out, offs, nfiles, ids, starts, seed, mode);
  return hipGetLastError();
}

__global__ void rebase_files_kernel(pfscdc_segment* __restrict__ segs, uint64_t n, uint32_t base) {
  for (uint64_t i = blockIdx.x * (uint64_t)blockDim.x + threadIdx.x; i < n;
       i += (uint64_t)gridDim.x * blockDim.x)
    segs[i].file += base;
}

hipError_t launch_rebase_files(pfscdc_segment* segs, uint64_t n, uint32_t base, hipStream_t st) {
  if (n == 0 || base == 0) return hipSuccess;
  const uint64_t blocks = std::min<uint64_t>((n + 255) / 256, 1024);
  rebase_files_kernel<<<(unsigned)blocks, 256, 0, st>>>(segs, n, base);
  return hipGetLastError();
}

}
```

### pfs_amd/csrc/knobs.cpp

```cpp
#include <atomic>
#include <cerrno>
#include <cstdio>
#include <cstdlib>
#include <cstring>

#include <unistd.h>

#include "pfscdc_internal.h"

namespace pfscdc {
namespace {

struct KnobDef {
  const char* name;
  int64_t def, lo, hi;
};

constexpr int64_t kMax = (int64_t)1 << 62;
constexpr KnobDef kDefs[(int)Knob::kCount] = {
    {"PFSCDC_SCAN_SKIP", 1, 0, 1},
    {"PFSCDC_SCAN_CUTSKIP", 1, 0, 1},
    {"PFSCDC_SCAN_GRID", 0, 0, 1 << 20},
    {"PFSCDC_HASH_GRID", 0, 0, 1 << 20},
    {"PFSCDC_CHACHA_GRID", 0, 0, 1 << 20},
    {"PFSCDC_HASH_BIN_BYTES", -1, -1, kMax},
    {"PFSCDC_HASH_WAVES", 0, 0, 8},
    {"PFSCDC_HASH_FAIR", 1, 0, 1},
    {"PFSCDC_HASH_FAIR_EVERY", 256, 8, 65536},
    {"PFSCDC_REFID_SPLIT", -1, -1, 1},
    {"PFSCDC_COMMIT_TWO_SETS", -1, -1, 1},
    {"PFSCDC_COMMIT_LONG_PCT", 30, 1, 99},
    {"PFSCDC_UW_WORKERS", 1, 1, 8},
    {"PFSCDC_UW_INFLIGHT", (int64_t)32 << 30, 0, kMax},
    {"PFSCDC_UW_MIRROR", 1, 0, 1},
    {"PFSCDC_UW_INDEX_GROUPED", 1, 0, 1},
    {"PFSCDC_UW_ARENA_POOL_BYTES", 40000000000ll, 0, kMax},
    {"PFSCDC_CTX_CACHE", 32, 0, 4096},
    {"PFSCDC_COPY_THREADS", 0, 0, 256},
    {"PFSCDC_INDEX_DECODE", 1, 0, 1},
    {"PFSCDC_INDEX_MERGE", 0, 0, 1},
    {"PFSCDC_SOURCE", 1, 0, 1},
    {"PFSCDC_DIFF", 1, 0, 1},
    {"PFSCDC_COPY_MAP", 1, 0, 1},
    {"PFSCDC_TRACE", 0, 0, 1},
};

static_assert(kDefs[(int)Knob::kCount - 1].name != nullptr, "one entry per Knob");

struct Table {
  std::atomic<int64_t> v[(int)Knob::kCount];
  std::atomic<bool> frozen[(int)Knob::kCount];
  Table() {
    for (auto& f : frozen) f.store(false, std::memory_order_relaxed);
    for (int i = 0; i < (int)Knob::kCount; i++) {
      const KnobDef& d = kDefs[i];
      int64_t x = d.def;
      const char* e = std::getenv(d.name);
      if (e && *e) {
        char* end = nullptr;
        errno = 0;
        const long long y = std::strtoll(e, &end, 10);
        if (errno || !end || *end || y < d.lo || y > d.hi)
          std::fprintf(stderr, "pfscdc: ignoring %s=%s (want an integer in [%lld, %lld])\n",
                       d.name, e, (long long)d.lo, (long long)d.hi);
        else
          x = y;
      }
      v[i].store(x, std::memory_order_relaxed);
    }
    for (char** e = environ; e && *e; e++) {
      if (std::strncmp(*e, "PFSCDC_", 7) != 0) continue;
      const char* eq = std::strchr(*e, '=');
      const size_t len = eq ? (size_t)(eq - *e) : std::strlen(*e);
      bool known = false;
      for (int i = 0; i < (int)Knob::kCount && !known; i++)
        known = std::strlen(kDefs[i].name) == len && std::strncmp(kDefs[i].name, *e, len) == 0;
      if (!known)
        std::fprintf(stderr, "pfscdc: ignoring %.*s (not a knob of this library; "
                     "INTEGRATION.md lists them)\n", (int)len, *e);
    }
  }
};

Table& table() {
  static Table* t = new Table();
  return *t;
}

int find(const char* name) {
  if (!name) return -1;
  for (int i = 0; i < (int)Knob::kCount; i++)
    if (std::strcmp(kDefs[i].name, name) == 0) return i;
  return -1;
}

}

int64_t knob(Knob k) { return table().v[(int)k].load(std::memory_order_relaxed); }

int64_t knob_freeze(Knob k) {
  table().frozen[(int)k].store(true, std::memory_order_relaxed);
  return knob(k);
}

}

extern "C" {

int pfscdc_set_knob(const char* name, int64_t value) {
  const int i = pfscdc::find(name);
  if (i < 0) return PFSCDC_EINVAL;
// ... 28 lines not shown
```

### pfs_amd/csrc/pfscdc.cpp

```cpp
#include <hip/hip_runtime.h>

#include <algorithm>
#include <cstdio>
#include <cstring>
#include <string>
#include <vector>

#include <unistd.h>

#include "dev_list.h"
#include "pfscdc_internal.h"

using namespace pfscdc;

namespace {

template <typename T>
struct DevBuf {
  T* p = nullptr;
  size_t cap = 0;
  hipError_t ensure(size_t n, bool exact = false) {
    if (n <= cap && p) return hipSuccess;
    if (p) (void)hipFree(p);
    p = nullptr;
    cap = 0;
    size_t want = std::max<size_t>(n, 1);
    if (!exact) want = want + want / 4;
    hipError_t e = hipMalloc((void**)&p, want * sizeof(T));
    if (e == hipSuccess) cap = want;
    return e;
  }
  void release() {
    if (p) (void)hipFree(p);
    p = nullptr;
    cap = 0;
  }
};

template <typename T>
struct PinnedBuf {
  T* p = nullptr;
  size_t cap = 0;
  hipError_t ensure(size_t n) {
    if (n <= cap && p) return hipSuccess;
    if (p) (void)hipHostFree(p);
    p = nullptr;
    cap = 0;
    size_t want = std::max<size_t>(n, 1);
    want = want + want / 4;
    hipError_t e = hipHostMalloc((void**)&p, want * sizeof(T), hipHostMallocDefault);
    if (e == hipSuccess) cap = want;
    return e;
  }
  void release() {
    if (p) (void)hipHostFree(p);
    p = nullptr;
    cap = 0;
  }
};

struct CreatePending {
  bool active = false, split = false;
  uint32_t k = 0, nr = 0;
  uint8_t* hashes = nullptr;
  pfscdc_ref* refs = nullptr;
};

}

struct pfscdc_ctx {
  pfscdc_params params{};
  int device = 0;
  int num_cus = 256;
  hipStream_t own_stream = nullptr;
  hipStream_t stream = nullptr;
  std::string err;
  uint64_t table[256];
  uint64_t* d_table = nullptr;
  DevBuf<uint8_t> d_data, d_tail;
  DevBuf<TileRec> d_recs;
  DevBuf<uint32_t> d_unit_ctr;
  DevBuf<uint32_t> d_skip;
  DevBuf<uint32_t> d_uinfo, d_plan;
  DevBuf<uint4> d_uslots;
  DevBuf<uint32_t> d_rslots;
  DevBuf<ScanPlan> d_planhdr;
  bool scan_skipped = false;
  uint32_t scan_mode = 0;
  uint64_t scanned_bytes = 0;
  bool cuts_only = false;
  DevBuf<uint64_t> d_entries, d_counts;
  DevBuf<uint64_t> d_offs, d_seg_base, d_nseg, d_seg_begin;
  DevBuf<pfscdc_segment> d_slots, d_segs;
  DevBuf<uint32_t> d_order, d_qctr;
  DevBuf<uint32_t> d_next;
  uint64_t bin_bytes = 0;
  DevBuf<pfscdc_ref> d_refs;
  DevBuf<uint8_t> d_out;
  DevBuf<uint64_t> d_span;
  PinnedBuf<uint64_t> h_span;
  double wall_khz = 100000.0;
  DevBuf<uint32_t> d_ids;
  DevBuf<uint64_t> d_starts;
  DevBuf<uint8_t> d_group, d_group_ct;
  DevBuf<pfscdc_segment> d_segs2;
  DevBuf<uint64_t> d_blk;
  DevBuf<uint8_t> d_ctext;
  PinnedBuf<uint64_t> h_blk;
  PinnedBuf<pfscdc_segment> h_segs2;
  PinnedBuf<pfscdc_ref> h_refs;
  DevBuf<pfscdc_slice> d_rslices;
  DevBuf<uint64_t> d_rmeta;
  DevBuf<uint8_t> d_rok;
  PinnedBuf<pfscdc_slice> h_rslices;
  PinnedBuf<uint64_t> h_rmeta;
  PinnedBuf<uint8_t> h_rok;
  DevBuf<TarEntry> d_tar;
  DevBuf<uint8_t> d_tnames;
  PinnedBuf<TarEntry> h_tar;
  PinnedBuf<uint8_t> h_tnames;
  DevBuf<uint64_t> d_txblk;
  PinnedBuf<uint64_t> h_txblk;
  int tar_format = PFSCDC_TAR_USTAR;
  hipEvent_t rev[4] = {nullptr, nullptr, nullptr, nullptr};
  float read_ms[2] = {0.f, 0.f};
  float frame_ms = 0.f;
  uint32_t options = 0;
  float get_ms = 0.f;
  float create_ms = 0.f, create_hash_ms = 0.f;
  int create_form = -1;
  hipEvent_t cev = nullptr;
  hipEvent_t wev = nullptr;
  hipStream_t aux_stream = nullptr;
  hipEvent_t xev[2] = {nullptr, nullptr};
  std::vector<uint32_t> perm;
  CreatePending cr;
  int cr_wave_cap = 0;
  uint32_t cr_hash_prio = 0;
  bool cr_chacha_prio = false;
  bool cr_one_stream = false;
  pfscdc_ctx* helper = nullptr;
  hipEvent_t pev[3] = {nullptr, nullptr, nullptr};
  bool have_refs = false;
  bool scan_valid = false;
  bool host_records = true;
  PinnedBuf<uint64_t> h_offs, h_seg_base, h_seg_begin;
  PinnedBuf<pfscdc_segment> h_segs;
  hipEvent_t ev[8] = {};
  bool pending = false;
  uint32_t nfiles = 0;
  uint64_t nbytes = 0;
  uint64_t ntiles = 0;
  uint64_t slot_cap = 0;
  uint64_t nsegs = 0;
  const uint8_t* dev_data = nullptr;
  pfscdc_ctx* hash_after = nullptr;
  IndexStats index_stats;
  MergeStats merge_stats;
  ResidentStats resident_stats;
  PassStats source_stats;
  PassStats diff_stats;
  PassStats copy_map_stats;
};

namespace pfscdc {
const pfscdc_params& ctx_params(const pfscdc_ctx* ctx) { return ctx->params; }
IndexStats& ctx_index_stats(pfscdc_ctx* ctx) { return ctx->index_stats; }
MergeStats& ctx_merge_stats(pfscdc_ctx* ctx) { return ctx->merge_stats; }
ResidentStats& ctx_resident_stats(pfscdc_ctx* ctx) { return ctx->resident_stats; }
PassStats& ctx_source_stats(pfscdc_ctx* ctx) { return ctx->source_stats; }
PassStats& ctx_diff_stats(pfscdc_ctx* ctx) { return ctx->diff_stats; }
PassStats& ctx_copy_map_stats(pfscdc_ctx* ctx) { return ctx->copy_map_stats; }
int ctx_num_cus(const pfscdc_ctx* ctx) { return ctx->num_cus; }
int ctx_tar_format(const pfscdc_ctx* ctx) { return ctx->tar_format; }
}

namespace {

static int scan_grid(uint64_t ntiles, int num_cus) {
// ... 61 lines not shown
    return hipMemcpyAsync(u->d_segs.p, u->h_segs.p, sizeof(pfscdc_segment) * n,
                          hipMemcpyHostToDevice, st);
  }
  hipError_t upload_counts(hipStream_t st, uint32_t counts = 1) const {
    if (counts == 1) u->h_seg_begin.p[0] = n;
    return hipMemcpyAsync(u->d_counts.p + 1, u->h_seg_begin.p, counts * sizeof(uint64_t),
                          hipMemcpyHostToDevice, st);
  }
  hipError_t upload(hipStream_t st, uint32_t counts = 1) const {
    hipError_t e = upload_offsets(st);
    if (e == hipSuccess) e = upload_records(st);
    if (e == hipSuccess) e = upload_counts(st, counts);
    return e;
  }
  hipError_t hash(const uint8_t* data, uint64_t nbytes, hipStream_t st, int wave_cap = 0,
                  uint32_t prio = 0) const {
    int w = knob_waves(longest, sum, u->num_cus);
    if (wave_cap > 0 && w > wave_cap) w = wave_cap;
    return launch_blake2b(data, u->d_offs.p, u->d_segs.p, u->d_counts.p + 1, n, u->d_order.p,
                          u->d_qctr.p, u->num_cus, nbytes, st, false, nullptr, w, prio);
  }
  hipError_t download(hipStream_t st) const {
    if (!n) return hipSuccess;
    return hipMemcpyAsync(u->h_segs.p, u->d_segs.p, sizeof(pfscdc_segment) * n,
                          hipMemcpyDeviceToHost, st);
  }
};

int check_chunk_offsets(pfscdc_ctx* c, const uint64_t* chunk_offsets, uint32_t nchunks,
                        uint64_t nbytes) {
  if (chunk_offsets[0] != 0 || chunk_offsets[nchunks] != nbytes)
    return fail(c, PFSCDC_EINVAL, "chunk_offsets must start at 0 and end at nbytes");
  for (uint32_t i = 0; i < nchunks; i++)
    if (chunk_offsets[i + 1] < chunk_offsets[i])
      return fail(c, PFSCDC_EINVAL, "chunk_offsets must be nondecreasing");
  return PFSCDC_OK;
}

int check_device_arg(pfscdc_ctx* c, const void* p, int on_device, const char* what) {
  if (on_device && ((uintptr_t)p & 15))
    return fail(c, PFSCDC_EINVAL, std::string("device ") + what + " must be 16-byte aligned");
  return PFSCDC_OK;
}

hipError_t stage_in(pfscdc_ctx* c, const void* bytes, uint64_t nbytes, int on_device,
                    hipStream_t st, const uint8_t** data) {
  *data = (const uint8_t*)bytes;
  if (on_device) return hipSuccess;
  hipError_t e = c->d_data.ensure(nbytes + 64);
  *data = c->d_data.p;
  if (e == hipSuccess && nbytes)
    e = hipMemcpyAsync(c->d_data.p, bytes, nbytes, hipMemcpyHostToDevice, st);
  return e;
}

hipError_t stage_out(pfscdc_ctx* c, void* out, uint64_t nbytes, int on_device, uint8_t** outp) {
  *outp = (uint8_t*)out;
  if (on_device) return hipSuccess;
  const hipError_t e = c->d_out.ensure(nbytes + 64);
  *outp = c->d_out.p;
  return e;
}

int validate_params(const pfscdc_params* p, std::string* why) {
  if (!p) {
    *why = "params is NULL";
    return PFSCDC_EINVAL;
  }
  if (p->average_bits < 1 || p->average_bits > 63) {
    *why = "average_bits must be in [1, 63]";
    return PFSCDC_EINVAL;
  }
  if (p->max_chunk < p->min_chunk || p->min_chunk < 1) {
    *why = "need 1 <= min_chunk <= max_chunk";
    return PFSCDC_EINVAL;
  }
  if (p->min_chunk < 64) {
    *why = "min_chunk < 64 (the rolling window) is not supported on the GPU path";
    return PFSCDC_EUNSUPPORTED;
  }
  return PFSCDC_OK;
}

constexpr int kSpanSlots = 8;
hipError_t reset_spans(pfscdc_ctx* c, hipStream_t st) {
  hipError_t e = hipMemsetAsync(c->d_span.p, 0, kSpanSlots * sizeof(uint64_t), st);
  if (e == hipSuccess) e = hipMemsetAsync(c->d_span.p, 0xFF, sizeof(uint64_t), st);
  if (e == hipSuccess) e = hipMemsetAsync(c->d_span.p + 2, 0xFF, sizeof(uint64_t), st);
  return e;
}

}

extern "C" {

void pfscdc_default_params(pfscdc_params* p) {
  p->average_bits = 23;
  p->reserved = 0;
  p->seed = 1;
  p->min_chunk = 1000000;
  p->max_chunk = 20000000;
}

int pfscdc_table(int64_t seed, uint64_t out[256]) {
  if (!out) return PFSCDC_EINVAL;
  generate_hashes(seed, out);
  return PFSCDC_OK;
}

int pfscdc_go_int63(int64_t seed, int64_t* out, int n) {
  if (!out || n < 0) return PFSCDC_EINVAL;
  go_int63(seed, out, n);
  return PFSCDC_OK;
}

int pfscdc_ctx_create(const pfscdc_params* params, int device, pfscdc_ctx** out) {
  return pfscdc::ctx_create_on(params, device, nullptr, out);
}

}

int pfscdc::ctx_create_on(const pfscdc_params* params, int device, hipStream_t shared,
                          pfscdc_ctx** out) {
  if (!out) return PFSCDC_EINVAL;
  *out = nullptr;
  std::string why;
  int rc = validate_params(params, &why);
  if (rc) {
    std::fprintf(stderr, "pfscdc_ctx_create: %s\n", why.c_str());
    return rc;
  }
  int ndev = 0;
  if (hipGetDeviceCount(&ndev) != hipSuccess || ndev == 0) {
    std::fprintf(stderr, "pfscdc_ctx_create: no HIP device visible\n");
    return PFSCDC_EHIP;
  }
  if (device < 0 || device >= ndev) return PFSCDC_EINVAL;
  pfscdc_ctx* c = new pfscdc_ctx();
  c->params = *params;
  c->device = device;
  if (hipSetDevice(device) != hipSuccess) {
    delete c;
    return PFSCDC_EHIP;
  }
  hipDeviceProp_t prop;
  if (hipGetDeviceProperties(&prop, device) == hipSuccess) c->num_cus = prop.multiProcessorCount;
  int khz = 0;
  if (hipDeviceGetAttribute(&khz, hipDeviceAttributeWallClockRate, device) == hipSuccess && khz > 0)
    c->wall_khz = khz;
  if (hipError_t e = prepare_kernels(); e != hipSuccess) {
    std::fprintf(stderr, "pfscdc_ctx_create: kernel attributes: %s\n", hipGetErrorString(e));
    delete c;
    return PFSCDC_EHIP;
  }
  generate_hashes(params->seed, c->table);
  if ((!shared && hipStreamCreateWithFlags(&c->own_stream, hipStreamNonBlocking) != hipSuccess) ||
      hipMalloc((void**)&c->d_table, sizeof c->table) != hipSuccess ||
      hipMemcpy(c->d_table, c->table, sizeof c->table, hipMemcpyHostToDevice) != hipSuccess) {
    delete c;
    return PFSCDC_EHIP;
  }
  for (auto& e : c->ev)
    if (hipEventCreate(&e) != hipSuccess) {
      delete c;
      return PFSCDC_EHIP;
    }
  if (hipEventCreate(&c->cev) != hipSuccess ||
      hipEventCreateWithFlags(&c->wev, hipEventDisableTiming) != hipSuccess) {
    delete c;
    return PFSCDC_EHIP;
  }
  c->stream = shared ? shared : c->own_stream;
  *out = c;
  return PFSCDC_OK;
}

extern "C" {

int pfscdc_ctx_destroy(pfscdc_ctx* c) {
  if (!c) return PFSCDC_EINVAL;
  (void)hipSetDevice(c->device);
  if (c->pending) (void)hipStreamSynchronize(c->stream);
  if (c->helper) pfscdc_ctx_destroy(c->helper);
  c->d_data.release();
  c->d_tail.release();
  c->d_recs.release();
  c->d_unit_ctr.release();
  c->d_entries.release();
  c->d_skip.release();
  c->d_uinfo.release();
  c->d_plan.release();
  c->d_uslots.release();
  c->d_rslots.release();
  c->d_planhdr.release();
  c->d_counts.release();
  c->d_offs.release();
  c->d_seg_base.release();
  c->d_nseg.release();
  c->d_seg_begin.release();
  c->d_slots.release();
  c->d_segs.release();
  c->d_next.release();
  c->d_order.release();
  c->d_qctr.release();
  c->d_refs.release();
  c->h_refs.release();
  c->d_out.release();
  c->d_ids.release();
  c->d_span.release();
  c->h_span.release();
  c->d_starts.release();
  c->d_group.release();
  c->d_group_ct.release();
  c->d_segs2.release();
  c->d_blk.release();
  c->d_ctext.release();
  c->h_blk.release();
  c->h_segs2.release();
  c->h_offs.release();
  c->h_seg_base.release();
  c->h_seg_begin.release();
  c->h_segs.release();
  c->d_rslices.release();
  c->d_rmeta.release();
  c->d_rok.release();
  c->h_rslices.release();
  c->h_rmeta.release();
  c->h_rok.release();
  c->d_tar.release();
  c->d_tnames.release();
  c->h_tar.release();
  c->h_tnames.release();
  c->d_txblk.release();
  c->h_txblk.release();
  for (auto& e : c->rev)
    if (e) (void)hipEventDestroy(e);
  if (c->d_table) (void)hipFree(c->d_table);
  for (auto& e : c->ev)
    if (e) (void)hipEventDestroy(e);
  if (c->cev) (void)hipEventDestroy(c->cev);
  if (c->wev) (void)hipEventDestroy(c->wev);
  if (c->own_stream) (void)hipStreamDestroy(c->own_stream);
  if (c->aux_stream) (void)hipStreamDestroy(c->aux_stream);
  for (auto& e : c->pev)
    if (e) (void)hipEventDestroy(e);
  for (auto& e : c->xev)
    if (e) (void)hipEventDestroy(e);
  delete c;
  return PFSCDC_OK;
}

const char* pfscdc_last_error(const pfscdc_ctx* c) { return c ? c->err.c_str() : "null ctx"; }

int pfscdc_set_stream(pfscdc_ctx* c, void* hip_stream) {
  if (!c) return PFSCDC_EINVAL;
  c->stream = hip_stream ? (hipStream_t)hip_stream : c->own_stream;
  return PFSCDC_OK;
}

int pfscdc_order_hash_after(pfscdc_ctx* c, pfscdc_ctx* other) {
  if (!c || other == c) return PFSCDC_EINVAL;
  c->hash_after = other;
  return PFSCDC_OK;
}

void* pfscdc_stream_handle(const pfscdc_ctx* c) { return c ? (void*)c->stream : nullptr; }

int pfscdc_stream_wait(pfscdc_ctx* c, void* hip_stream) {
  if (!c) return PFSCDC_EINVAL;
  hipStream_t s = (hipStream_t)hip_stream;
  if (s == c->stream) return PFSCDC_OK;
  PFS_HIP(c, hipSetDevice(c->device));
  PFS_HIP(c, hipEventRecord(c->wev, s));
  PFS_HIP(c, hipStreamWaitEvent(c->stream, c->wev, 0));
  return PFSCDC_OK;
}

}

namespace {

#define HIP_OK(ctx, expr) PFS_HIP(ctx, expr)

int scan_async_impl(pfscdc_ctx* c, const void* bytes, uint64_t nbytes, int bytes_on_device,
                    const uint64_t* file_offsets, uint32_t nfiles, uint32_t options) {
  if (!c) return PFSCDC_EINVAL;
  if (c->pending) return fail(c, PFSCDC_ESTATE, "previous scan not waited for");
  c->cuts_only = false;
  if (!file_offsets) return fail(c, PFSCDC_EINVAL, "file_offsets is NULL");
  if (nbytes && !bytes) return fail(c, PFSCDC_EINVAL, "bytes is NULL");
  if (file_offsets[0] != 0 || file_offsets[nfiles] != nbytes)
    return fail(c, PFSCDC_EINVAL, "file_offsets must start at 0 and end at nbytes");
  for (uint32_t f = 0; f < nfiles; f++)
    if (file_offsets[f + 1] < file_offsets[f])
      return fail(c, PFSCDC_EINVAL, "file_offsets must be nondecreasing");
  if (bytes_on_device && ((uintptr_t)bytes & 15))
    return fail(c, PFSCDC_EINVAL, "device bytes must be 16-byte aligned");
  c->ntiles = (nbytes + kTile - 1) / kTile;
  if (c->ntiles * (uint64_t)kScanWaves >= (1ull << 32))
    return fail(c, PFSCDC_EUNSUPPORTED, "batch too large for one scan (split it)");
  c->scan_valid = false;
  HIP_OK(c, hipSetDevice(c->device));
  hipStream_t st = c->stream;
  const pfscdc_params& p = c->params;

  HIP_OK(c, c->h_offs.ensure(nfiles + 1));
  HIP_OK(c, c->h_seg_base.ensure(nfiles + 1));
  std::memcpy(c->h_offs.p, file_offsets, sizeof(uint64_t) * (nfiles + 1));
  uint64_t cap = 0, longest_file = 0;
  for (uint32_t f = 0; f < nfiles; f++) {
    c->h_seg_base.p[f] = cap;
    const uint64_t len = file_offsets[f + 1] - file_offsets[f];
    cap += len ? len / (uint64_t)p.min_chunk + 1 : 0;
    longest_file = std::max(longest_file, len);
  }
  const int waves = knob_waves(std::min<uint64_t>(longest_file, (uint64_t)p.max_chunk), nbytes,
                              c->num_cus);
  const uint64_t quads = (uint64_t)c->num_cus * 4 * (uint64_t)waves * 16;
  const int64_t kb = knob(Knob::HashBinBytes);
  const uint64_t bin_bytes = kb >= 0 ? (uint64_t)kb : (nbytes + quads - 1) / quads;
  c->h_seg_base.p[nfiles] = cap;
  c->bin_bytes = bin_bytes;
  c->slot_cap = cap;
  c->nfiles = nfiles;
  c->nbytes = nbytes;

  HIP_OK(c, c->d_offs.ensure(nfiles + 1));
  HIP_OK(c, c->d_seg_base.ensure(nfiles + 1));
  HIP_OK(c, c->d_nseg.ensure(nfiles + 1));
  HIP_OK(c, c->d_seg_begin.ensure(nfiles + 1));
  HIP_OK(c, c->d_slots.ensure(cap));
  HIP_OK(c, c->d_segs.ensure(cap));
  HIP_OK(c, c->d_order.ensure(cap));
  if (bin_bytes) HIP_OK(c, c->d_next.ensure(cap));
  HIP_OK(c, c->d_qctr.ensure(2));
  if (options & PFSCDC_OPT_REF_IDS) HIP_OK(c, c->d_refs.ensure(cap));
  HIP_OK(c, c->d_recs.ensure(c->ntiles));
  HIP_OK(c, c->d_unit_ctr.ensure(3));
  HIP_OK(c, c->d_entries.ensure(c->ntiles * kTileK + 1));
  HIP_OK(c, c->d_counts.ensure(7));
  HIP_OK(c, c->d_tail.ensure(kTailBytes));
  HIP_OK(c, c->d_span.ensure(kSpanSlots));
  HIP_OK(c, c->h_span.ensure(kSpanSlots + 4));

  const uint8_t* data;
  if (bytes_on_device) {
    data = (const uint8_t*)bytes;
  } else {
    HIP_OK(c, c->d_data.ensure(nbytes + 64));
    if (nbytes) HIP_OK(c, hipMemcpyAsync(c->d_data.p, bytes, nbytes, hipMemcpyHostToDevice, st));
    data = c->d_data.p;
  }
  c->dev_data = data;
  HIP_OK(c, hipMemcpyAsync(c->d_offs.p, c->h_offs.p, sizeof(uint64_t) * (nfiles + 1),
                           hipMemcpyHostToDevice, st));
  HIP_OK(c, hipMemcpyAsync(c->d_seg_base.p, c->h_seg_base.p, sizeof(uint64_t) * (nfiles + 1),
                           hipMemcpyHostToDevice, st));
  const uint64_t n_main = nbytes & ~63ULL;
  HIP_OK(c, hipMemsetAsync(c->d_tail.p, 0, kTailBytes, st));
  if (nbytes > n_main)
    HIP_OK(c, hipMemcpyAsync(c->d_tail.p, data + n_main, nbytes - n_main,
                             hipMemcpyDeviceToDevice, st));
  HIP_OK(c, hipMemsetAsync(c->d_counts.p, 0, 7 * sizeof(uint64_t), st));
  if (c->ntiles) HIP_OK(c, hipMemsetAsync(c->d_recs.p, 0, sizeof(TileRec) * c->ntiles, st));
  HIP_OK(c, hipMemsetAsync(c->d_unit_ctr.p, 0, 3 * sizeof(uint32_t), st));
  HIP_OK(c, reset_spans(c, st));

  HIP_OK(c, hipEventRecord(c->ev[0], st));
  c->scan_skipped = false;
  c->scan_mode = 0;
  if (c->ntiles) {
    const uint32_t* skip = nullptr;
    c->scan_skipped = knob(Knob::ScanSkip) != 0;
    c->scan_mode = c->scan_skipped ? PFSCDC_SCAN_SKIPPED_FIRST_MIN : 0u;
    const ScanPlan* d_plan = nullptr;
    const uint64_t nunits = c->ntiles * kScanWaves;
    if (c->scan_skipped) {
      HIP_OK(c, c->d_skip.ensure(nunits));
      const bool cs_room = nfiles < kPlanMaxFiles &&
                           (uint64_t)nfiles * kRankSlots * sizeof(uint32_t) * 64 <= nbytes;
      if (cs_room && cut_skip_exact(p)) {
        c->scan_mode |= PFSCDC_SCAN_SKIPPED_CUTS;
        HIP_OK(c, c->d_uinfo.ensure(2 * nunits));
        HIP_OK(c, c->d_uslots.ensure(nunits));
        HIP_OK(c, c->d_plan.ensure(kPlanWords));
        HIP_OK(c, c->d_rslots.ensure((size_t)nfiles * kRankSlots));
        HIP_OK(c, hipMemsetAsync(c->d_plan.p, 0, kPlanWords * sizeof(uint32_t), st));
        HIP_OK(c, hipMemsetAsync(c->d_rslots.p, 0, (size_t)nfiles * kRankSlots * sizeof(uint32_t), st));
        HIP_OK(c, c->d_planhdr.ensure(1));
        const ScanPlan hdr{c->d_uslots.p, c->d_plan.p, c->d_uinfo.p, c->d_rslots.p, c->d_offs.p,
                           (uint64_t)p.min_chunk, (uint64_t)p.max_chunk,
                           (unsigned long long*)(c->d_counts.p + 6)};
        HIP_OK(c, launch_scan_plan(c->d_offs.p, nfiles, nbytes, (uint64_t)p.min_chunk, c->ntiles,
                                   c->d_skip.p, c->d_counts.p + 3, c->d_uinfo.p, c->d_uslots.p,
                                   c->d_plan.p, hdr, c->d_planhdr.p, st));
        d_plan = c->d_planhdr.p;
      } else {
        HIP_OK(c, launch_scan_skip(c->d_offs.p, nfiles, nbytes, (uint64_t)p.min_chunk, c->ntiles,
                                   c->d_skip.p, c->d_counts.p + 3, st));
      }
      skip = c->d_skip.p;
    }
    const int grid = scan_grid(c->ntiles, c->num_cus);
    HIP_OK(c, launch_scan(data, c->d_tail.p, nbytes, c->d_table, p.average_bits, c->ntiles,
                          c->d_recs.p, grid, c->d_unit_ctr.p, c->d_unit_ctr.p + 1,
                          c->d_entries.p, c->d_counts.p, c->d_span.p, st, skip, d_plan));
  }
  HIP_OK(c, hipEventRecord(c->ev[1], st));
  HIP_OK(c, hipEventRecord(c->ev[2], st));
  if (nfiles)
    HIP_OK(c, launch_select(data, c->d_table, c->d_entries.p, c->d_counts.p, c->d_offs.p,
                            c->d_seg_base.p, nfiles, p.average_bits, (uint64_t)p.min_chunk,
                            (uint64_t)p.max_chunk, c->d_slots.p, c->d_nseg.p,
                            c->d_unit_ctr.p + 2, c->d_segs.p, c->d_seg_begin.p, c->d_order.p,
                            c->d_qctr.p, st, bin_bytes, bin_bytes ? c->d_next.p : nullptr,
                            c->d_counts.p + 4));
  const uint64_t* qlen = c->d_counts.p + 4;
  const uint32_t* next = bin_bytes ? c->d_next.p : nullptr;
  HIP_OK(c, hipEventRecord(c->ev[3], st));
  if (c->hash_after && c->hash_after->device == c->device)
    HIP_OK(c, hipStreamWaitEvent(st, c->hash_after->ev[4], 0));
  if (nfiles && !(options & kScanNoHash))
    HIP_OK(c, launch_blake2b(data, c->d_offs.p, c->d_segs.p, qlen, cap,
                             c->d_order.p, c->d_qctr.p, c->num_cus, nbytes, st, true,
                             c->d_span.p + 2, waves, 0u, waves == 1, next,
                             knob(Knob::HashFair) && waves > 1 && next ? c->d_counts.p + 5
                                                                      : nullptr,
                             (uint32_t)knob(Knob::HashFairEvery)));
  HIP_OK(c, hipEventRecord(c->ev[4], st));
  c->have_refs = (options & PFSCDC_OPT_REF_IDS) != 0 && !(options & kScanNoHash);
  if (c->have_refs && nfiles)
    HIP_OK(c, launch_ref_ids(data, c->d_offs.p, c->d_segs.p, qlen, cap,
                             c->d_order.p, c->d_qctr.p + 1, c->num_cus, nbytes, c->d_refs.p,
                             nullptr, st, waves, 0u, next, c->d_seg_begin.p + nfiles));
  HIP_OK(c, hipEventRecord(c->ev[6], st));
  HIP_OK(c, c->h_seg_begin.ensure(nfiles + 1));
  if (nfiles)
    HIP_OK(c, hipMemcpyAsync(c->h_seg_begin.p, c->d_seg_begin.p, sizeof(uint64_t) * (nfiles + 1),
                             hipMemcpyDeviceToHost, st));
  else
    c->h_seg_begin.p[0] = 0;
  c->pending = true;
  return PFSCDC_OK;
}

#undef HIP_OK

}

extern "C" {

int pfscdc_scan_async(pfscdc_ctx* c, const void* bytes, uint64_t nbytes, int bytes_on_device,
                      const uint64_t* file_offsets, uint32_t nfiles) {
  if (!c) return PFSCDC_EINVAL;
  const uint32_t o = c->options;
  const bool cuts = (o & PFSCDC_OPT_CUTS_ONLY) != 0;
  const int rc = scan_async_impl(c, bytes, nbytes, bytes_on_device, file_offsets, nfiles,
                                 (o & ~PFSCDC_OPT_CUTS_ONLY) | (cuts ? kScanNoHash : 0u));
  if (rc == PFSCDC_OK) c->cuts_only = cuts;
  return rc;
}

int pfscdc_wait(pfscdc_ctx* c) { return pfscdc::wait_impl(c, true); }

}

int pfscdc::wait_impl(pfscdc_ctx* c, bool fetch) {
  if (!c) return PFSCDC_EINVAL;
  if (!c->pending) return PFSCDC_OK;
  c->pending = false;
  PFS_HIP(c, hipSetDevice(c->device));
  PFS_HIP(c, hipStreamSynchronize(c->stream));
  const uint64_t total = c->nfiles ? c->h_seg_begin.p[c->nfiles] : 0;
  if (total > c->slot_cap) return fail(c, PFSCDC_EHIP, "segment count exceeds slot capacity");
  PFS_HIP(c, c->h_segs.ensure(total));
  if (total && fetch)
    PFS_HIP(c, hipMemcpyAsync(c->h_segs.p, c->d_segs.p, total * sizeof(pfscdc_segment),
                              hipMemcpyDeviceToHost, c->stream));
  if (c->have_refs && fetch) {
    PFS_HIP(c, c->h_refs.ensure(total));
    if (total)
      PFS_HIP(c, hipMemcpyAsync(c->h_refs.p, c->d_refs.p, total * sizeof(pfscdc_ref),
                                hipMemcpyDeviceToHost, c->stream));
  }
  PFS_HIP(c, hipMemcpyAsync(c->h_span.p, c->d_span.p, kSpanSlots * sizeof(uint64_t),
                            hipMemcpyDeviceToHost, c->stream));
  const bool skipped = c->scan_skipped && c->ntiles;
  if (skipped)
    PFS_HIP(c, hipMemcpyAsync(c->h_span.p + kSpanSlots, c->d_counts.p + 3, 4 * sizeof(uint64_t),
                              hipMemcpyDeviceToHost, c->stream));
  PFS_HIP(c, hipEventRecord(c->ev[5], c->stream));
  PFS_HIP(c, hipStreamSynchronize(c->stream));
  c->scanned_bytes = skipped ? c->h_span.p[kSpanSlots] - c->h_span.p[kSpanSlots + 3] : c->nbytes;
  c->nsegs = total;
  c->scan_valid = fetch;
  c->host_records = fetch;
  return PFSCDC_OK;
}

extern "C" {

int pfscdc_last_kernel_spans(pfscdc_ctx* c, float out[2]) {
  if (!c || !out) return PFSCDC_EINVAL;
  if (c->pending) return fail(c, PFSCDC_ESTATE, "scan pending");
  if (!c->h_span.p) {
    out[0] = out[1] = 0.f;
    return PFSCDC_OK;
  }
  const double ticks_per_ms = c->wall_khz;
  for (int k = 0; k < 2; k++) {
    const uint64_t a = c->h_span.p[2 * k], b = c->h_span.p[2 * k + 1];
    out[k] = (b > a && a != ~0ULL) ? (float)((double)(b - a) / ticks_per_ms) : 0.f;
  }
  return PFSCDC_OK;
}

int pfscdc_last_kernel_clocks(pfscdc_ctx* c, float out[2]) {
  if (!c || !out) return PFSCDC_EINVAL;
  if (c->pending) return fail(c, PFSCDC_ESTATE, "scan pending");
  out[0] = out[1] = 0.f;
  if (!c->h_span.p) return PFSCDC_OK;
  for (int k = 0; k < 2; k++) {
    const uint64_t cyc = c->h_span.p[4 + 2 * k], ticks = c->h_span.p[5 + 2 * k];
    out[k] = ticks ? (float)((double)cyc / (double)ticks * (c->wall_khz / 1000.0)) : 0.f;
  }
  return PFSCDC_OK;
}

int pfscdc_scan(pfscdc_ctx* c, const void* bytes, uint64_t nbytes, int bytes_on_device,
                const uint64_t* file_offsets, uint32_t nfiles) {
  int rc = pfscdc_scan_async(c, bytes, nbytes, bytes_on_device, file_offsets, nfiles);
  if (rc) return rc;
  return pfscdc_wait(c);
}

uint64_t pfscdc_num_segments(const pfscdc_ctx* c) { return c ? c->nsegs : 0; }

int pfscdc_set_options(pfscdc_ctx* c, uint32_t options) {
  if (!c || (options & ~(PFSCDC_OPT_REF_IDS | PFSCDC_OPT_CUTS_ONLY | PFSCDC_OPT_CTEXT_IN_PLACE)))
    return PFSCDC_EINVAL;
  if (c->pending) return fail(c, PFSCDC_ESTATE, "set_options during a pending scan");
// ... 10 lines not shown
  *ms = 0.f;
  if (c->have_refs) PFS_HIP(c, hipEventElapsedTime(ms, c->ev[4], c->ev[6]));
  return PFSCDC_OK;
}
const pfscdc_segment* pfscdc_segments(const pfscdc_ctx* c) {
  return c && c->host_records ? c->h_segs.p : nullptr;
}
const uint64_t* pfscdc_file_segment_begin(const pfscdc_ctx* c) {
  return c ? c->h_seg_begin.p : nullptr;
}

uint64_t pfscdc_debug_candidates(pfscdc_ctx* c, uint64_t* out, uint64_t cap) {
  if (!c || c->pending || !c->ntiles) return 0;
  uint64_t ne = 0;
  if (hipMemcpy(&ne, c->d_counts.p, sizeof ne, hipMemcpyDeviceToHost) != hipSuccess) return 0;
  if (out && cap) {
    const uint64_t k = std::min(ne, cap);
    if (hipMemcpy(out, c->d_entries.p, k * sizeof(uint64_t), hipMemcpyDeviceToHost) != hipSuccess)
      return 0;
  }
  return ne;
}

uint64_t pfscdc_debug_hash_queue(pfscdc_ctx* c, uint32_t* order, uint64_t order_cap,
                                 uint32_t* next, uint64_t next_cap, uint64_t* bin_bytes) {
  if (bin_bytes) *bin_bytes = 0;
  if (!c || c->pending || !c->scan_valid || !c->nfiles) return 0;
  if (bin_bytes) *bin_bytes = c->bin_bytes;
  if (hipSetDevice(c->device) != hipSuccess) return 0;
  uint64_t qlen = 0;
  if (hipMemcpy(&qlen, c->d_counts.p + 4, sizeof qlen, hipMemcpyDeviceToHost) != hipSuccess)
    return 0;
  const uint64_t k = std::min(std::min(qlen, order_cap), c->slot_cap);
  if (order && k &&
      hipMemcpy(order, c->d_order.p, k * sizeof(uint32_t), hipMemcpyDeviceToHost) != hipSuccess)
    return 0;
  const uint64_t m = c->bin_bytes ? std::min(c->nsegs, next_cap) : 0;
  if (next && m &&
      hipMemcpy(next, c->d_next.p, m * sizeof(uint32_t), hipMemcpyDeviceToHost) != hipSuccess)
    return 0;
  return qlen;
}

uint64_t pfscdc_debug_scan_plan(pfscdc_ctx* c, uint32_t* slots, uint64_t cap) {
  if (!c || c->pending || !c->ntiles || !(c->scan_mode & PFSCDC_SCAN_SKIPPED_CUTS)) return 0;
  if (hipSetDevice(c->device) != hipSuccess) return 0;
  uint32_t ns = 0;
  if (hipMemcpy(&ns, c->d_plan.p, sizeof ns, hipMemcpyDeviceToHost) != hipSuccess) return 0;
  const uint64_t k = std::min<uint64_t>(std::min<uint64_t>(ns, cap), c->ntiles * kScanWaves);
  if (slots && k) {
    std::vector<uint4> h(k);
    if (hipMemcpy(h.data(), c->d_uslots.p, k * sizeof(uint4), hipMemcpyDeviceToHost) != hipSuccess)
      return 0;
    for (uint64_t i = 0; i < k; i++) {
      slots[3 * i] = h[i].x;
      slots[3 * i + 1] = h[i].y;
      slots[3 * i + 2] = h[i].z;
    }
  }
  return ns;
}

int pfscdc_last_scan_bytes(pfscdc_ctx* c, uint64_t* out) {
  if (!c || !out) return PFSCDC_EINVAL;
  if (c->pending) return fail(c, PFSCDC_ESTATE, "scan pending");
  *out = c->scanned_bytes;
  return PFSCDC_OK;
}

int pfscdc_last_scan_mode(pfscdc_ctx* c, uint32_t* mode) {
  if (!c || !mode) return PFSCDC_EINVAL;
  if (c->pending) return fail(c, PFSCDC_ESTATE, "scan pending");
  *mode = c->scan_mode;
  return PFSCDC_OK;
}

int pfscdc_last_timings(pfscdc_ctx* c, float out[5]) {
  if (!c || !out) return PFSCDC_EINVAL;
  PFS_HIP(c, hipEventElapsedTime(&out[0], c->ev[0], c->ev[1]));
  PFS_HIP(c, hipEventElapsedTime(&out[1], c->ev[1], c->ev[2]));
  PFS_HIP(c, hipEventElapsedTime(&out[2], c->ev[2], c->ev[3]));
  PFS_HIP(c, hipEventElapsedTime(&out[3], c->ev[3], c->ev[4]));
  PFS_HIP(c, hipEventElapsedTime(&out[4], c->ev[0], c->ev[4]));
  return PFSCDC_OK;
}

int pfscdc_get_chunks(pfscdc_ctx* c, const void* ctext, uint64_t nbytes, int ctext_on_device,
                      const uint64_t* chunk_offsets, uint32_t nchunks, const pfscdc_ref* refs,
                      void* ptext, int ptext_on_device, uint8_t* ok) {
  if (!c) return PFSCDC_EINVAL;
  if (c->pending) return fail(c, PFSCDC_ESTATE, "get_chunks during a pending scan");
  if (!chunk_offsets || (nchunks && (!refs || !ok)) || (nbytes && (!ctext || !ptext)))
    return fail(c, PFSCDC_EINVAL, "NULL argument");
  if (int rc = check_chunk_offsets(c, chunk_offsets, nchunks, nbytes)) return rc;
  if (int rc = check_device_arg(c, ctext, ctext_on_device, "ctext")) return rc;
  if (nchunks == 0) return PFSCDC_OK;
  scan_overwritten(c);
  PFS_HIP(c, hipSetDevice(c->device));
  hipStream_t st = c->stream;
  HashBatch b{c};
  PFS_HIP(c, b.reserve(nchunks, nchunks + 1));
  std::memcpy(c->h_offs.p, chunk_offsets, sizeof(uint64_t) * (nchunks + 1));
  for (uint32_t i = 0; i < nchunks; i++) b.add(i, 0, chunk_offsets[i + 1] - chunk_offsets[i]);
  PFS_HIP(c, c->h_refs.ensure(nchunks));
  std::memcpy(c->h_refs.p, refs, sizeof(pfscdc_ref) * nchunks);
  PFS_HIP(c, c->d_refs.ensure(nchunks));
  const uint8_t* in;
  uint8_t* outp;
  PFS_HIP(c, stage_in(c, ctext, nbytes, ctext_on_device, st, &in));
  PFS_HIP(c, stage_out(c, ptext, nbytes, ptext_on_device, &outp));
  PFS_HIP(c, b.upload_offsets(st));
  PFS_HIP(c, b.upload_records(st));
  PFS_HIP(c, hipMemcpyAsync(c->d_refs.p, c->h_refs.p, sizeof(pfscdc_ref) * nchunks,
                            hipMemcpyHostToDevice, st));
  PFS_HIP(c, b.upload_counts(st));
  PFS_HIP(c, hipEventRecord(c->ev[7], st));
  PFS_HIP(c, launch_get(in, c->d_offs.p, c->d_segs.p, c->d_counts.p + 1, nchunks, c->d_order.p,
                        c->d_qctr.p, c->num_cus, nbytes, c->d_refs.p, outp, st,
                        knob_waves(b.longest, nbytes, c->num_cus)));
  PFS_HIP(c, hipEventRecord(c->ev[6], st));
  PFS_HIP(c, b.download(st));
  if (!ptext_on_device && nbytes)
    PFS_HIP(c, hipMemcpyAsync(ptext, outp, nbytes, hipMemcpyDeviceToHost, st));
  PFS_HIP(c, hipStreamSynchronize(st));
  for (uint32_t i = 0; i < nchunks; i++)
    ok[i] = std::memcmp(c->h_segs.p[i].hash, refs[i].id, 32) == 0 ? 1 : 0;
  float ms = 0.f;
  if (hipEventElapsedTime(&ms, c->ev[7], c->ev[6]) == hipSuccess) c->get_ms = ms;
  return PFSCDC_OK;
}

int pfscdc_create_refs(pfscdc_ctx* c, const void* bytes, uint64_t nbytes, int bytes_on_device,
                       const uint64_t* chunk_offsets, uint32_t nchunks, uint8_t* content_hashes,
                       const uint8_t* hash_known, pfscdc_ref* refs) {
  if (!c) return PFSCDC_EINVAL;
  if (c->pending) return fail(c, PFSCDC_ESTATE, "create_refs during a pending scan");
  if (!chunk_offsets || (nchunks && !refs) || (nbytes && !bytes) || (hash_known && !content_hashes))
    return fail(c, PFSCDC_EINVAL, "NULL argument");
  if (int rc = check_chunk_offsets(c, chunk_offsets, nchunks, nbytes)) return rc;
  if (int rc = check_device_arg(c, bytes, bytes_on_device, "bytes")) return rc;
  if (nchunks == 0) return PFSCDC_OK;
  PFS_HIP(c, hipSetDevice(c->device));
  const uint8_t* data;
  PFS_HIP(c, stage_in(c, bytes, nbytes, bytes_on_device, c->stream, &data));
  return create_refs_device(c, data, nbytes, chunk_offsets, nchunks, content_hashes, hash_known,
                            refs);
}

constexpr int kOnePass = 1;

static bool commit_two_sets(uint32_t nchunks, int num_cus) {
  const int64_t k = knob(Knob::CommitTwoSets);
  if (k >= 0) return k != 0;
  return (uint64_t)nchunks > (uint64_t)num_cus * 4 * 16;
}

static int commit_refs_two_sets(pfscdc_ctx* c, const uint8_t* data, uint64_t nbytes,
                                const std::vector<uint64_t>& sbeg, const std::vector<uint64_t>& ssz,
                                const uint64_t* co, uint32_t nchunks, uint8_t* content_hashes,
                                const uint8_t* hash_known, pfscdc_ref* refs,
                                uint8_t* segment_hashes, uint8_t* ct) {
  if (!commit_two_sets(nchunks, c->num_cus) || nchunks < 2) return kOnePass;
  const uint64_t m = sbeg.size();
  std::vector<uint32_t> seg_chunk(m);
  std::vector<int64_t> known_seg(nchunks, -1);
  for (uint64_t s = 0; s < m; s++) {
// ... 982 lines not shown
```

### pfs_amd/csrc/pfscdc_internal.h

```cpp
#pragma once
#include <hip/hip_runtime.h>
#include <stdint.h>

#include <string>
#include <vector>

#include "../../include/pfscdc.h"
#include "tar.h"

namespace pfscdc {

constexpr int kScanWaves = 12;
constexpr int kScanBlock = 64 * kScanWaves;
constexpr int kStrip = 4096;
constexpr uint64_t kTile = (uint64_t)kScanBlock * kStrip;
constexpr int kTileK = 15;
constexpr uint32_t kTableLdsBytes = 256u * 256u;
constexpr uint32_t kStageBytes = 64u * 128u;
constexpr uint32_t kScanLdsBytes = kTableLdsBytes + kScanWaves * kStageBytes;
static_assert(kScanLdsBytes <= 160 * 1024, "scan kernel LDS budget");
constexpr int kCompactBlock = 1024;
constexpr int kSelectBlock = 1024;
constexpr int kHashBlock = 256;
constexpr int kHashWavesPerSimd = 2;
constexpr uint64_t kDenseBit = 1ULL << 63;
constexpr uint64_t kNone = ~0ULL;
constexpr uint32_t kNoNext = 0xffffffffu;
constexpr uint64_t kTailBytes = 256;

struct TileRec {
  uint32_t count;
  uint32_t off[kTileK];
};
static_assert(sizeof(TileRec) == 64, "tile record is one 64-byte line");
static_assert(sizeof(pfscdc_segment) == 56, "segment record layout");
static_assert(sizeof(pfscdc_ref) == 64, "ref record layout");
static_assert(sizeof(pfscdc_slice) == 24, "slice record layout");

enum class Knob : int {
  ScanSkip, ScanCutSkip, ScanGrid, HashGrid, ChachaGrid,
  HashBinBytes, HashWaves, HashFair, HashFairEvery,
  RefIdSplit, CommitTwoSets, CommitLongPct,
  UwWorkers, UwInflight, UwMirror, UwIndexGrouped, UwArenaPoolBytes, CtxCache, CopyThreads,
  IndexDecode, IndexMerge, Source, Diff, CopyMap, Trace,
  kCount
};
int64_t knob(Knob k);
int64_t knob_freeze(Knob k);
inline unsigned capped_grid(uint64_t grid, Knob cap_knob) {
  const int64_t cap = knob(cap_knob);
  if (cap > 0 && (uint64_t)cap < grid) grid = (uint64_t)cap;
  return (unsigned)grid;
}

void generate_hashes(int64_t seed, uint64_t out[256]);
const pfscdc_params& ctx_params(const pfscdc_ctx* ctx);
void go_int63(int64_t seed, int64_t* out, int n);

constexpr uint32_t kScanNoHash = 0x100;
int hash_records_device(pfscdc_ctx* ctx, const uint8_t* data, uint64_t nbytes,
                        const uint64_t* begins, const uint64_t* sizes, uint32_t n, uint8_t* out);
int scan_sync(pfscdc_ctx* ctx, const void* bytes, uint64_t nbytes, int bytes_on_device,
              const uint64_t* file_offsets, uint32_t nfiles, uint32_t options);
int create_refs_device(pfscdc_ctx* ctx, const uint8_t* data, uint64_t nbytes,
                       const uint64_t* offs, uint32_t n, uint8_t* hashes, const uint8_t* known,
                       pfscdc_ref* refs, uint8_t* ctext_out = nullptr,
                       const uint32_t* sel = nullptr, uint32_t nsel = 0, bool finish = true);
int create_refs_finish(pfscdc_ctx* ctx);
int ctx_create_on(const pfscdc_params* params, int device, hipStream_t shared, pfscdc_ctx** out);
int ctx_device(const pfscdc_ctx* ctx);
hipError_t ctx_group_buffers(pfscdc_ctx* ctx, uint64_t bytes, bool ctext, uint8_t** d,
                             uint8_t** dct);
int writers_close_group(pfscdc_writer* const* ws, size_t n, double* stage_ms = nullptr,
                        const hipEvent_t* wait_events = nullptr, size_t n_wait = 0);
int writer_write_span(pfscdc_writer* w, const uint8_t* p, uint64_t n,
                      const uint8_t* dev = nullptr);
void writer_drop_prefetched(pfscdc_writer* w);
uint32_t ctx_options(const pfscdc_ctx* ctx);
bool ctx_scan_valid(const pfscdc_ctx* ctx);
uint32_t ctx_nfiles(const pfscdc_ctx* ctx);
uint64_t ctx_file_offset(const pfscdc_ctx* ctx, uint32_t f);
int wait_impl(pfscdc_ctx* ctx, bool fetch);
void ctx_device_results(const pfscdc_ctx* ctx, pfscdc_segment** segs, pfscdc_ref** refs,
                        uint64_t* n);
hipStream_t ctx_stream(const pfscdc_ctx* ctx);

hipError_t prepare_kernels();

constexpr uint64_t kScanUnit = 64ull * kStrip;
constexpr uint64_t kUnitStep = 64ull * 128;
constexpr uint32_t kUnitSteps = kStrip / 128;
constexpr uint32_t kPlanBuckets = 64;
constexpr uint32_t kPlanWords = 2 + kPlanBuckets;
constexpr uint32_t kPlanMaxFiles = 1u << 24;
constexpr uint32_t kRankSlots = 64;
constexpr uint32_t kSlotDone = 1u << 31;
struct ScanPlan {
  const uint4* slots;
  const uint32_t* plan;
  const uint32_t* uinfo;
  uint32_t* rslots;
  const uint64_t* offs;
  uint64_t min_chunk, max_chunk;
  unsigned long long* dyn_skipped;
};
hipError_t launch_scan(const uint8_t* data, const uint8_t* tail, uint64_t n, const uint64_t* d_table,
                       uint32_t average_bits, uint64_t ntiles, TileRec* recs, int grid,
                       uint32_t* unit_ctr, uint32_t* done_ctr, uint64_t* entries,
                       uint64_t* n_entries, uint64_t* span, hipStream_t st,
                       const uint32_t* skip = nullptr, const ScanPlan* d_plan = nullptr);
hipError_t launch_scan_skip(const uint64_t* offs, uint32_t nfiles, uint64_t n, uint64_t min_chunk,
                            uint64_t ntiles, uint32_t* skip, uint64_t* scanned, hipStream_t st);
hipError_t launch_scan_plan(const uint64_t* offs, uint32_t nfiles, uint64_t n, uint64_t min_chunk,
                            uint64_t ntiles, uint32_t* skip, uint64_t* scanned, uint32_t* uinfo,
                            uint4* slots, uint32_t* plan, const ScanPlan& hdr, ScanPlan* d_hdr,
                            hipStream_t st);
hipError_t launch_select(const uint8_t* data, const uint64_t* d_table, const uint64_t* entries,
                         const uint64_t* n_entries, const uint64_t* offs,
                         const uint64_t* seg_base, uint32_t nfiles, uint32_t average_bits,
                         uint64_t min_chunk, uint64_t max_chunk, pfscdc_segment* slots,
                         uint64_t* nseg, uint32_t* done_ctr, pfscdc_segment* segs,
                         uint64_t* seg_begin, uint32_t* order, uint32_t* counter,
                         hipStream_t st, uint64_t bin_bytes = 0, uint32_t* next = nullptr,
                         uint64_t* qlen = nullptr);
constexpr uint32_t kHashPrioAuto = 0x3fffffffu;
constexpr uint32_t kHashPrioNone = 0x80000000u;
hipError_t launch_blake2b(const uint8_t* data, const uint64_t* offs, pfscdc_segment* segs,
                          const uint64_t* seg_count, uint64_t max_segments, uint32_t* order,
                          uint32_t* counter, int num_cus, uint64_t nbytes, hipStream_t st,
                          bool ordered = false, uint64_t* span = nullptr, int waves = 0,
                          uint32_t prio = 0,
                          bool cu_exclusive = false,
                          const uint32_t* next = nullptr,
                          uint64_t* fair = nullptr,
                          uint32_t fair_every = 256);
int hash_waves(uint64_t longest_bytes, uint64_t total_bytes, int num_cus, int forced);
hipError_t launch_order(const pfscdc_segment* segs, const uint64_t* seg_count, uint32_t* order,
                        uint32_t* counter, hipStream_t st);
hipError_t launch_ref_ids(const uint8_t* data, const uint64_t* offs, pfscdc_segment* segs,
                          const uint64_t* seg_count, uint64_t max_segments, const uint32_t* order,
                          uint32_t* counter, int num_cus, uint64_t nbytes, pfscdc_ref* refs,
                          uint8_t* ctext_out, hipStream_t st, int waves = 0, uint32_t prio = 0,
                          const uint32_t* next = nullptr,
                          const uint64_t* nsegs = nullptr);
hipError_t launch_deks(pfscdc_segment* segs, const uint64_t* seg_count, uint64_t max_segments,
                       pfscdc_ref* refs, uint32_t* counter, hipStream_t st);
hipError_t launch_chacha_xor(const uint8_t* data, const uint64_t* offs, const pfscdc_segment* segs,
                             const uint64_t* blk_base, uint32_t n, uint64_t nblocks,
                             const pfscdc_ref* refs, uint8_t* out, int num_cus, hipStream_t st,
                             bool prio = false, bool one_wave_per_simd = false);
hipError_t launch_get(const uint8_t* ctext, const uint64_t* offs, pfscdc_segment* segs,
                      const uint64_t* seg_count, uint64_t nsegs, uint32_t* order, uint32_t* counter,
                      int num_cus, uint64_t nbytes, pfscdc_ref* refs, uint8_t* ptext, hipStream_t st,
                      int waves = 0);
hipError_t launch_verify_ids(const pfscdc_segment* segs, uint32_t n, const pfscdc_ref* refs,
                             uint8_t* ok, hipStream_t st);
hipError_t launch_slice_gather(const uint8_t* ctext, const uint64_t* chunk_offs,
                               const pfscdc_ref* refs, const uint8_t* ok,
                               const pfscdc_slice* slices, const uint64_t* out_off,
                               const uint64_t* blk_base, uint32_t n, uint64_t nblocks,
                               uint8_t* out, int num_cus, hipStream_t st);
hipError_t launch_tar_frame(const TarEntry* d_entries, const uint8_t* d_names, uint32_t n,
                            const uint64_t* d_xblk, uint64_t nx, uint64_t begin, uint64_t end,
                            uint64_t total, uint8_t* out, int num_cus, hipStream_t st);
int ctx_fail(pfscdc_ctx* ctx, int code, const std::string& msg);
#define PFS_HIP(ctx, expr)                                                             \
  do {                                                                                 \
    hipError_t e_ = (expr);                                                            \
    if (e_ != hipSuccess)                                                              \
      return pfscdc::ctx_fail(ctx, e_ == hipErrorOutOfMemory ? PFSCDC_ENOMEM : PFSCDC_EHIP, \
                              std::string(#expr) + ": " + hipGetErrorString(e_));      \
  } while (0)
int read_slices_impl(pfscdc_ctx* ctx, const void* ctext, uint64_t nbytes, int ctext_on_device,
                     const uint64_t* chunk_offsets, uint32_t nchunks, const pfscdc_ref* refs,
                     const uint8_t* verified, const pfscdc_slice* slices, uint32_t nslices,
                     void* out, int out_on_device, uint8_t* chunk_ok, uint8_t* slice_ok,
                     bool strict, const TarPlan* tar = nullptr);
struct DevSlices {
  const pfscdc_slice* slices;
  const uint64_t *out_off, *blk_base;
  uint32_t m;
  uint64_t nblocks;
};
struct DevTar {
  const TarEntry* entries;
  const uint8_t* names;
  uint32_t nent;
  uint64_t begin, end, total;
  const uint64_t* xblk;
  uint64_t nx;
};
int read_slices_dev_impl(pfscdc_ctx* ctx, const void* ctext, uint64_t nbytes,
                         const uint64_t* chunk_offsets, uint32_t nchunks, const pfscdc_ref* refs,
                         const DevSlices& sl, void* out, int out_on_device, uint8_t* chunk_ok,
                         const DevTar& tar, uint64_t* h2d_bytes, uint64_t* d2h_bytes);
hipError_t launch_rebase_files(pfscdc_segment* segs, uint64_t n, uint32_t base, hipStream_t st);
int ctx_num_cus(const pfscdc_ctx* ctx);
int ctx_tar_format(const pfscdc_ctx* ctx);
struct IndexStats {
  uint64_t n[4] = {};
  float ms[5] = {};
};
IndexStats& ctx_index_stats(pfscdc_ctx* ctx);
struct MergeStats {
  uint64_t n[4] = {};
  float ms[4] = {};
};
MergeStats& ctx_merge_stats(pfscdc_ctx* ctx);
struct PassStats {
  uint64_t n[8] = {};
  float ms[4] = {};
};
PassStats& ctx_source_stats(pfscdc_ctx* ctx);
PassStats& ctx_diff_stats(pfscdc_ctx* ctx);
PassStats& ctx_copy_map_stats(pfscdc_ctx* ctx);
struct RtarRun {
  pfscdc_ref ref;
  int64_t ref_size;
// ... 16 lines not shown
```

Measured before the change: 1329.

## Hash file prefixes concurrently with the CDC scan on a side stream

New measurement: 1329. Within noise of the previous version (-0.1%).

```diff
diff --git a/include/pfscdc.h b/include/pfscdc.h
--- a/include/pfscdc.h
+++ b/include/pfscdc.h
@@ -149,6 +149,7 @@
 int pfscdc_last_timings(pfscdc_ctx* ctx, float out[5]);
 int pfscdc_last_kernel_spans(pfscdc_ctx* ctx, float out[2]);
 int pfscdc_last_kernel_clocks(pfscdc_ctx* ctx, float out[2]);
+int pfscdc_last_prefix_timings(pfscdc_ctx* ctx, float out[2]);
 
 void* pfscdc_host_alloc(uint64_t nbytes);
 void pfscdc_host_free(void* p);
diff --git a/pfs_amd/_lib.py b/pfs_amd/_lib.py
--- a/pfs_amd/_lib.py
+++ b/pfs_amd/_lib.py
@@ -50,6 +50,7 @@
     "pfscdc_merge_file_hash", "pfscdc_last_create_timings", "pfscdc_last_create_form", "pfscdc_writer_prefetch",
     "pfscdc_candidates", "pfscdc_hash_ranges", "pfscdc_fill_synthetic_pieces",
     "pfscdc_last_kernel_spans", "pfscdc_last_kernel_clocks", "pfscdc_order_hash_after",
+    "pfscdc_last_prefix_timings",
     "pfscdc_set_knob", "pfscdc_get_knob", "pfscdc_knob_info", "pfscdc_last_scan_mode",
     "pfscdc_deal", "pfscdc_group_create", "pfscdc_group_destroy", "pfscdc_group_size",
     "pfscdc_group_ctx", "pfscdc_group_last_error", "pfscdc_group_scan",
@@ -276,6 +277,7 @@
             "pfscdc_get_knob": (i32, [C.c_char_p, P(i64)]),
             "pfscdc_knob_info": (C.c_char_p, [i32, P(i64), P(i64), P(i64)]),
             "pfscdc_last_kernel_spans": (i32, [vp, P(C.c_float)]),
+            "pfscdc_last_prefix_timings": (i32, [vp, P(C.c_float)]),
             "pfscdc_last_kernel_clocks": (i32, [vp, P(C.c_float)]),
             "pfscdc_set_options": (i32, [vp, u32]),
             "pfscdc_refs": (vp, [vp]),
diff --git a/pfs_amd/cdc.py b/pfs_amd/cdc.py
--- a/pfs_amd/cdc.py
+++ b/pfs_amd/cdc.py
@@ -169,6 +169,9 @@
         ck = (C.c_float * 2)()
         self._check(self.lib.pfscdc_last_kernel_clocks(self.ctx, ck), "kernel_clocks")
         t["scan_mhz"], t["hash_mhz"] = ck[0], ck[1]
+        pf = (C.c_float * 2)()
+        self._check(self.lib.pfscdc_last_prefix_timings(self.ctx, pf), "prefix_timings")
+        t["prefix"], t["prefix_span"] = pf[0], pf[1]
         if self.ref_ids:
             ms = C.c_float()
             self._check(self.lib.pfscdc_last_ref_ms(self.ctx, C.byref(ms)), "timings")
diff --git a/pfs_amd/csrc/cdc_kernels.hip b/pfs_amd/csrc/cdc_kernels.hip
--- a/pfs_amd/csrc/cdc_kernels.hip
+++ b/pfs_amd/csrc/cdc_kernels.hip
@@ -695,19 +695,23 @@
                              uint32_t* __restrict__ order, uint32_t* __restrict__ counter,
                              uint32_t* hist, uint64_t* s_wave,
                              const uint64_t* __restrict__ offs = nullptr, uint64_t bin_bytes = 0,
-                             uint32_t* __restrict__ next = nullptr, uint64_t* qlen = nullptr) {
+                             uint32_t* __restrict__ next = nullptr, uint64_t* qlen = nullptr,
+                             uint64_t pfx_min = 0, uint64_t pfx_bytes = 0) {
   const bool bins = next && offs && bin_bytes;
+  auto done_of = [&](uint32_t f) {
+    return pfx_bytes && offs[f + 1] - offs[f] >= pfx_min ? pfx_bytes : 0;
+  };
   auto binned = [&](uint64_t i) {
     const uint32_t f = segs[i].file;
-    return bins && offs[f + 1] - offs[f] <= bin_bytes;
+    return bins && offs[f + 1] - offs[f] - done_of(f) <= bin_bytes;
   };
   auto entry = [&](uint64_t i, uint32_t& key) {
     if (binned(i)) {
       const uint32_t f = segs[i].file;
-      key = lpt_key(offs[f + 1] - offs[f]);
+      key = lpt_key(offs[f + 1] - offs[f] - done_of(f));
       return i == 0 || segs[i - 1].file != f;
     }
-    key = lpt_key(segs[i].size);
+    key = lpt_key(segs[i].size - (pfx_bytes && segs[i].offset == 0 ? done_of(segs[i].file) : 0));
     return true;
   };
   constexpr int kPer = 1024 / BLOCK;
@@ -856,7 +860,7 @@
     pfscdc_segment* __restrict__ slots, uint64_t* __restrict__ nseg, uint32_t* done_ctr,
     pfscdc_segment* __restrict__ segs, uint64_t* __restrict__ seg_begin,
     uint32_t* __restrict__ order, uint32_t* __restrict__ counter, uint64_t bin_bytes,
-    uint32_t* __restrict__ next, uint64_t* __restrict__ qlen) {
+    uint32_t* __restrict__ next, uint64_t* __restrict__ qlen, uint64_t pfx_bytes) {
   __shared__ uint32_t hist[1024];
   __shared__ uint64_t s_wave[kSelectBlock / 64 + 1];
   __shared__ uint32_t s_flag;
@@ -871,7 +875,7 @@
   __syncthreads();
   if (order)
     lpt_order_block<kSelectBlock>(segs, total, order, counter, hist, s_wave, offs, bin_bytes,
-                                  next, qlen);
+                                  next, qlen, min_chunk, pfx_bytes);
 }
 
 
@@ -1174,7 +1178,7 @@
   hb = ((uint64_t)hbh << 32) | hbl;
 }
 
-constexpr int kModeHash = 0, kModeRefId = 1, kModeGet = 2;
+constexpr int kModeHash = 0, kModeRefId = 1, kModeGet = 2, kModePrefix = 3;
 template <int MODE>
 __global__ __launch_bounds__(kHashBlock) __attribute__((amdgpu_waves_per_eu(1, 2))) void blake2b_kernel(
     const uint8_t* __restrict__ data, const uint64_t* __restrict__ offs,
@@ -1182,15 +1186,16 @@
     const uint32_t* __restrict__ order, uint32_t* __restrict__ counter, uint64_t nbytes,
     pfscdc_ref* __restrict__ refs, uint8_t* __restrict__ out, uint32_t prio_blocks,
     uint64_t* span, const uint32_t* __restrict__ next, uint64_t* __restrict__ fair,
-    uint32_t fair_every) {
-  constexpr bool CIPHER = MODE != kModeHash;
+    uint32_t fair_every, uint64_t* mid, uint64_t pfx_min, uint32_t pfx_blocks, uint32_t nfiles) {
+  constexpr bool CIPHER = MODE == kModeRefId || MODE == kModeGet;
   const SpanClock span_clk = span_begin(span);
   constexpr uint32_t kMsgStride = 160, kMsgBuf = kHashBlock / 4 * kMsgStride;
   __shared__ __attribute__((aligned(16))) uint8_t s_msg[2 * kMsgBuf];
   const uint8_t* const end = data + nbytes;
   const uint32_t lane = threadIdx.x & 63u;
   const uint32_t j = lane & 3u;
-  const uint64_t nseg = *seg_count;
+  uint64_t nseg = nfiles;
+  if constexpr (MODE != kModePrefix) nseg = *seg_count;
   const uint32_t slot = (threadIdx.x >> 2) * kMsgStride;
   uint8_t* my = s_msg + slot + 32u * j;
 
@@ -1350,10 +1355,18 @@
         blk = 0;
         ha = h0a;
         hb = h0b;
+        if constexpr (MODE == kModeHash) {
+          if (mid && seg->offset == 0 && offs[seg->file + 1] - offs[seg->file] >= pfx_min) {
+            const uint64_t* ms = mid + (uint64_t)kMidStateWords * seg->file;
+            ha = ms[j];
+            hb = ms[4 + j];
+            blk = ms[8];
+          }
+        }
         active = true;
-        load_block(0);
+        load_block(blk);
         lds_put(cur);
-        if (nblk > 1) load_block(1);
+        if (nblk > blk + 1) load_block(blk + 1);
       };
       if (!active && bin_next != kNoNext) {
         begin(bin_next);
@@ -1475,21 +1488,115 @@
   };
   constexpr std::integral_constant<uint32_t, 0> P0{};
   constexpr std::integral_constant<uint32_t, 1> P1{};
-  while (true) {
-    if (!step(P0)) break;
-    if (!step(P1)) break;
-    wave_steps += 2;
-    if constexpr (MODE == kModeHash) {
-      if (quiet >= 5) {
-        uint64_t pre[4] = {lds_abs_u64(ma[0][0]), lds_abs_u64(ma[0][1]), lds_abs_u64(ma[0][2]),
-                           lds_abs_u64(ma[0][3])};
-        tm = ((blk + 1) << 7) & t_mask;
-        do {
+  if constexpr (MODE == kModePrefix) {
+    auto tail_step = [&](auto par, uint64_t* pre, bool fetch) {
+      constexpr uint32_t nxt = kMsgBuf - decltype(par)::value * kMsgBuf;
+      uint64_t a = ha, b = hb, c = iv_c, d = iv_d;
+      rounds(par, a, b, c, d, [&] {
+        if (active) {
+          lds_put(nxt);
+          if (fetch) msg_load_full(m0, m1, src + (blk + 2) * 128 + 32 * j);
+        }
+      }, pre, false, tm);
+      fold_diag(ha, hb, a, b, c, d);
+      tm += tinc;
+      blk++;
+    };
+    uint32_t file = 0;
+    while (true) {
+      active = false;
+      while (!drained) {
+        const bool need = !active;
+        const uint64_t want = __ballot(need && j == 0);
+        if (!want) break;
+        const uint32_t cnt = (uint32_t)__popcll(want);
+        const uint32_t leader = (uint32_t)__builtin_ctzll(want);
+        uint32_t base = 0;
+        if (lane == leader) base = atomicAdd(counter, cnt);
+        base = (uint32_t)__shfl((int)base, (int)leader, 64);
+        if (need) {
+          const uint64_t below = want & ((1ULL << (lane & ~3u)) - 1);
+          const uint64_t idx = (uint64_t)base + (uint64_t)__popcll(below);
+          if (idx < nseg && offs[idx + 1] - offs[idx] >= pfx_min) {
+            file = (uint32_t)idx;
+            src = data + offs[idx];
+            blk = 0;
+            ha = h0a;
+            hb = h0b;
+            active = true;
+            msg_load_full(m0, m1, src + 32 * j);
+            lds_put(0);
+            if (pfx_blocks > 1) msg_load_full(m0, m1, src + 128 + 32 * j);
+          }
+        }
+        if ((uint64_t)base + cnt >= nseg) drained = true;
+      }
+      if (__ballot(active) == 0) break;
+      __builtin_amdgcn_fence(__ATOMIC_RELEASE, "wavefront");
+      __builtin_amdgcn_wave_barrier();
+      __builtin_amdgcn_fence(__ATOMIC_ACQUIRE, "wavefront");
+      uint64_t pre[4] = {lds_abs_u64(ma[0][0]), lds_abs_u64(ma[0][1]), lds_abs_u64(ma[0][2]),
+                         lds_abs_u64(ma[0][3])};
+      tm = tinc;
+      uint32_t left = pfx_blocks;
+      while (left) {
+        if (fair) {
+          const uint32_t d = wave_steps - reported;
+          uint64_t tot = 0;
+          if (lane == 0) tot = atomicAdd((unsigned long long*)fair, (unsigned long long)d);
+          tot = ((uint64_t)__builtin_amdgcn_readfirstlane((uint32_t)(tot >> 32)) << 32) |
+                (uint32_t)__builtin_amdgcn_readfirstlane((uint32_t)tot);
+          reported = wave_steps;
+          if ((uint64_t)wave_steps * nwaves < tot + d) __builtin_amdgcn_s_setprio(1);
+          else __builtin_amdgcn_s_setprio(0);
+        }
+        uint32_t nfast = 0;
+        if (left >= 4) {
+          nfast = left - 2;
+          if (fair && nfast > kFairEvery) nfast = kFairEvery;
+          nfast &= ~1u;
+        }
+        for (uint32_t i = 0; i < nfast; i += 2) {
           fast_step(P0, pre);
           fast_step(P1, pre);
-          quiet -= 2;
-          wave_steps += 2;
-        } while (quiet >= 5);
+        }
+        left -= nfast;
+        wave_steps += nfast;
+        if (nfast == 0) {
+          tail_step(P0, pre, left >= 3);
+          left--;
+          wave_steps++;
+          if (left) {
+            tail_step(P1, pre, left >= 3);
+            left--;
+            wave_steps++;
+          }
+        }
+      }
+      if (active) {
+        uint64_t* ms = mid + (uint64_t)kMidStateWords * file;
+        ms[j] = ha;
+        ms[4 + j] = hb;
+        if (j == 0) ms[8] = pfx_blocks;
+      }
+    }
+  } else {
+    while (true) {
+      if (!step(P0)) break;
+      if (!step(P1)) break;
+      wave_steps += 2;
+      if constexpr (MODE == kModeHash) {
+        if (quiet >= 5) {
+          uint64_t pre[4] = {lds_abs_u64(ma[0][0]), lds_abs_u64(ma[0][1]), lds_abs_u64(ma[0][2]),
+                             lds_abs_u64(ma[0][3])};
+          tm = ((blk + 1) << 7) & t_mask;
+          do {
+            fast_step(P0, pre);
+            fast_step(P1, pre);
+            quiet -= 2;
+            wave_steps += 2;
+          } while (quiet >= 5);
+        }
       }
     }
   }
@@ -2107,7 +2214,8 @@
                          uint64_t min_chunk, uint64_t max_chunk, pfscdc_segment* slots,
                          uint64_t* nseg, uint32_t* done_ctr, pfscdc_segment* segs,
                          uint64_t* seg_begin, uint32_t* order, uint32_t* counter,
-                         hipStream_t st, uint64_t bin_bytes, uint32_t* next, uint64_t* qlen) {
+                         hipStream_t st, uint64_t bin_bytes, uint32_t* next, uint64_t* qlen,
+                         uint64_t pfx_bytes) {
   const uint64_t mask64 = average_bits >= 64 ? ~0ULL : ((1ULL << average_bits) - 1);
   const uint64_t waves_per_block = kSelectBlock / 64;
   const uint64_t grid = (nfiles + waves_per_block - 1) / waves_per_block;
@@ -2115,7 +2223,8 @@
                                                          offs, seg_base, nfiles, mask64,
                                                          min_chunk, max_chunk, slots, nseg,
                                                          done_ctr, segs, seg_begin, order,
-                                                         counter, bin_bytes, next, qlen);
+                                                         counter, bin_bytes, next, qlen,
+                                                         pfx_bytes);
   return hipGetLastError();
 }
 
@@ -2143,13 +2252,26 @@
                           uint32_t* counter, int num_cus, uint64_t nbytes, hipStream_t st,
                           bool ordered, uint64_t* span, int waves, uint32_t prio,
                           bool cu_exclusive, const uint32_t* next, uint64_t* fair,
-                          uint32_t fair_every) {
+                          uint32_t fair_every, const uint64_t* mid, uint64_t pfx_min) {
   if (max_segments == 0) return hipSuccess;
   if (!ordered) hash_order_kernel<<<1, kCompactBlock, 0, st>>>(segs, seg_count, order, counter);
   const size_t dyn = cu_exclusive ? 64u * 1024u : 0u;
   blake2b_kernel<kModeHash><<<hash_grid(max_segments, num_cus, waves), kHashBlock, dyn, st>>>(
       data, offs, segs, seg_count, order, counter, nbytes, nullptr, nullptr,
-      prio_arg(prio), span, ordered ? next : nullptr, ordered ? fair : nullptr, fair_every);
+      prio_arg(prio), span, ordered ? next : nullptr, ordered ? fair : nullptr, fair_every,
+      const_cast<uint64_t*>(mid), pfx_min, 0u, 0u);
+  return hipGetLastError();
+}
+
+hipError_t launch_blake2b_prefix(const uint8_t* data, const uint64_t* offs, uint32_t nfiles,
+                                 uint64_t nprefix, uint64_t pfx_min, uint32_t pfx_blocks,
+                                 uint64_t* mid, uint32_t* counter, int num_cus, uint64_t nbytes,
+                                 hipStream_t st, uint64_t* span, int waves, uint64_t* fair,
+                                 uint32_t fair_every) {
+  if (nprefix == 0 || pfx_blocks == 0) return hipSuccess;
+  blake2b_kernel<kModePrefix><<<hash_grid(nprefix, num_cus, waves), kHashBlock, 0, st>>>(
+      data, offs, nullptr, nullptr, nullptr, counter, nbytes, nullptr, nullptr, 0u, span, nullptr,
+      fair, fair_every, mid, pfx_min, pfx_blocks, nfiles);
   return hipGetLastError();
 }
 
@@ -2169,7 +2291,7 @@
       segs, nsegs ? nsegs : seg_count, refs, counter);
   blake2b_kernel<kModeRefId><<<hash_grid(max_segments, num_cus, waves), kHashBlock, 0, st>>>(
       data, offs, segs, seg_count, order, counter, nbytes, refs, ctext_out,
-      prio_arg(prio), nullptr, next, nullptr, 0u);
+      prio_arg(prio), nullptr, next, nullptr, 0u, nullptr, 0, 0u, 0u);
   return hipGetLastError();
 }
 
@@ -2201,7 +2323,7 @@
   hash_order_kernel<<<1, kCompactBlock, 0, st>>>(segs, seg_count, order, counter);
   blake2b_kernel<kModeGet><<<hash_grid(nsegs, num_cus, waves), kHashBlock, 0, st>>>(
       ctext, offs, segs, seg_count, order, counter, nbytes, refs, ptext, prio_arg(0), nullptr,
-      nullptr, nullptr, 0u);
+      nullptr, nullptr, 0u, nullptr, 0, 0u, 0u);
   return hipGetLastError();
 }
 
diff --git a/pfs_amd/csrc/knobs.cpp b/pfs_amd/csrc/knobs.cpp
--- a/pfs_amd/csrc/knobs.cpp
+++ b/pfs_amd/csrc/knobs.cpp
@@ -27,6 +27,7 @@
     {"PFSCDC_HASH_WAVES", 0, 0, 8},
     {"PFSCDC_HASH_FAIR", 1, 0, 1},
     {"PFSCDC_HASH_FAIR_EVERY", 256, 8, 65536},
+    {"PFSCDC_HASH_PREFIX", 1, 0, 1},
     {"PFSCDC_REFID_SPLIT", -1, -1, 1},
     {"PFSCDC_COMMIT_TWO_SETS", -1, -1, 1},
     {"PFSCDC_COMMIT_LONG_PCT", 30, 1, 99},
diff --git a/pfs_amd/csrc/pfscdc.cpp b/pfs_amd/csrc/pfscdc.cpp
--- a/pfs_amd/csrc/pfscdc.cpp
+++ b/pfs_amd/csrc/pfscdc.cpp
@@ -95,6 +95,12 @@
   DevBuf<uint32_t> d_order, d_qctr;
   DevBuf<uint32_t> d_next;
   uint64_t bin_bytes = 0;
+  hipStream_t pfx_stream = nullptr;
+  hipEvent_t pfx_fork = nullptr;
+  hipEvent_t pfx_ev[2] = {nullptr, nullptr};
+  DevBuf<uint64_t> d_mid;
+  DevBuf<uint32_t> d_pfx_ctr;
+  bool have_prefix = false;
   DevBuf<pfscdc_ref> d_refs;
   DevBuf<uint8_t> d_out;
   DevBuf<uint64_t> d_span;
@@ -322,11 +328,12 @@
   return PFSCDC_OK;
 }
 
-constexpr int kSpanSlots = 8;
+constexpr int kSpanSlots = 14;
 hipError_t reset_spans(pfscdc_ctx* c, hipStream_t st) {
   hipError_t e = hipMemsetAsync(c->d_span.p, 0, kSpanSlots * sizeof(uint64_t), st);
   if (e == hipSuccess) e = hipMemsetAsync(c->d_span.p, 0xFF, sizeof(uint64_t), st);
   if (e == hipSuccess) e = hipMemsetAsync(c->d_span.p + 2, 0xFF, sizeof(uint64_t), st);
+  if (e == hipSuccess) e = hipMemsetAsync(c->d_span.p + 8, 0xFF, sizeof(uint64_t), st);
   return e;
 }
 
@@ -441,6 +448,8 @@
   c->d_slots.release();
   c->d_segs.release();
   c->d_next.release();
+  c->d_mid.release();
+  c->d_pfx_ctr.release();
   c->d_order.release();
   c->d_qctr.release();
   c->d_refs.release();
@@ -482,6 +491,10 @@
   if (c->wev) (void)hipEventDestroy(c->wev);
   if (c->own_stream) (void)hipStreamDestroy(c->own_stream);
   if (c->aux_stream) (void)hipStreamDestroy(c->aux_stream);
+  if (c->pfx_stream) (void)hipStreamDestroy(c->pfx_stream);
+  if (c->pfx_fork) (void)hipEventDestroy(c->pfx_fork);
+  for (auto& e : c->pfx_ev)
+    if (e) (void)hipEventDestroy(e);
   for (auto& e : c->pev)
     if (e) (void)hipEventDestroy(e);
   for (auto& e : c->xev)
@@ -547,18 +560,26 @@
   HIP_OK(c, c->h_offs.ensure(nfiles + 1));
   HIP_OK(c, c->h_seg_base.ensure(nfiles + 1));
   std::memcpy(c->h_offs.p, file_offsets, sizeof(uint64_t) * (nfiles + 1));
-  uint64_t cap = 0, longest_file = 0;
+  uint64_t cap = 0, longest_file = 0, npfx = 0;
   for (uint32_t f = 0; f < nfiles; f++) {
     c->h_seg_base.p[f] = cap;
     const uint64_t len = file_offsets[f + 1] - file_offsets[f];
     cap += len ? len / (uint64_t)p.min_chunk + 1 : 0;
     longest_file = std::max(longest_file, len);
+    npfx += len >= (uint64_t)p.min_chunk;
   }
   const int waves = knob_waves(std::min<uint64_t>(longest_file, (uint64_t)p.max_chunk), nbytes,
                               c->num_cus);
   const uint64_t quads = (uint64_t)c->num_cus * 4 * (uint64_t)waves * 16;
+  const uint64_t pfx_blocks = ((uint64_t)p.min_chunk - 1) / 128;
+  const bool prefix = (options & kScanPrefix) && knob(Knob::HashPrefix) != 0 && waves > 1 &&
+                      !(options & (PFSCDC_OPT_REF_IDS | kScanNoHash)) && npfx > 0 &&
+                      pfx_blocks > 0 && pfx_blocks <= 0xffffffffull;
+  const uint64_t pfx_bytes = prefix ? 128 * pfx_blocks : 0;
+  c->have_prefix = false;
   const int64_t kb = knob(Knob::HashBinBytes);
-  const uint64_t bin_bytes = kb >= 0 ? (uint64_t)kb : (nbytes + quads - 1) / quads;
+  const uint64_t bin_bytes =
+      kb >= 0 ? (uint64_t)kb : (nbytes - npfx * pfx_bytes + quads - 1) / quads;
   c->h_seg_base.p[nfiles] = cap;
   c->bin_bytes = bin_bytes;
   c->slot_cap = cap;
@@ -574,11 +595,22 @@
   HIP_OK(c, c->d_order.ensure(cap));
   if (bin_bytes) HIP_OK(c, c->d_next.ensure(cap));
   HIP_OK(c, c->d_qctr.ensure(2));
+  if (prefix) {
+    HIP_OK(c, c->d_mid.ensure((size_t)nfiles * kMidStateWords));
+    HIP_OK(c, c->d_pfx_ctr.ensure(1));
+    if (!c->pfx_stream) {
+      int least = 0, greatest = 0;
+      HIP_OK(c, hipDeviceGetStreamPriorityRange(&least, &greatest));
+      HIP_OK(c, hipStreamCreateWithPriority(&c->pfx_stream, hipStreamNonBlocking, least));
+      HIP_OK(c, hipEventCreateWithFlags(&c->pfx_fork, hipEventDisableTiming));
+      for (auto& e : c->pfx_ev) HIP_OK(c, hipEventCreate(&e));
+    }
+  }
   if (options & PFSCDC_OPT_REF_IDS) HIP_OK(c, c->d_refs.ensure(cap));
   HIP_OK(c, c->d_recs.ensure(c->ntiles));
   HIP_OK(c, c->d_unit_ctr.ensure(3));
   HIP_OK(c, c->d_entries.ensure(c->ntiles * kTileK + 1));
-  HIP_OK(c, c->d_counts.ensure(7));
+  HIP_OK(c, c->d_counts.ensure(8));
   HIP_OK(c, c->d_tail.ensure(kTailBytes));
   HIP_OK(c, c->d_span.ensure(kSpanSlots));
   HIP_OK(c, c->h_span.ensure(kSpanSlots + 4));
@@ -601,12 +633,13 @@
   if (nbytes > n_main)
     HIP_OK(c, hipMemcpyAsync(c->d_tail.p, data + n_main, nbytes - n_main,
                              hipMemcpyDeviceToDevice, st));
-  HIP_OK(c, hipMemsetAsync(c->d_counts.p, 0, 7 * sizeof(uint64_t), st));
+  HIP_OK(c, hipMemsetAsync(c->d_counts.p, 0, 8 * sizeof(uint64_t), st));
   if (c->ntiles) HIP_OK(c, hipMemsetAsync(c->d_recs.p, 0, sizeof(TileRec) * c->ntiles, st));
   HIP_OK(c, hipMemsetAsync(c->d_unit_ctr.p, 0, 3 * sizeof(uint32_t), st));
   HIP_OK(c, reset_spans(c, st));
 
   HIP_OK(c, hipEventRecord(c->ev[0], st));
+  if (prefix) HIP_OK(c, hipEventRecord(c->pfx_fork, st));
   c->scan_skipped = false;
   c->scan_mode = 0;
   if (c->ntiles) {
@@ -646,6 +679,19 @@
                           c->d_recs.p, grid, c->d_unit_ctr.p, c->d_unit_ctr.p + 1,
                           c->d_entries.p, c->d_counts.p, c->d_span.p, st, skip, d_plan));
   }
+  if (prefix) {
+    hipStream_t ps = c->pfx_stream;
+    HIP_OK(c, hipStreamWaitEvent(ps, c->pfx_fork, 0));
+    HIP_OK(c, hipMemsetAsync(c->d_pfx_ctr.p, 0, sizeof(uint32_t), ps));
+    HIP_OK(c, hipEventRecord(c->pfx_ev[0], ps));
+    HIP_OK(c, launch_blake2b_prefix(data, c->d_offs.p, nfiles, npfx, (uint64_t)p.min_chunk,
+                                    (uint32_t)pfx_blocks, c->d_mid.p, c->d_pfx_ctr.p, c->num_cus,
+                                    nbytes, ps, c->d_span.p + 8, waves,
+                                    knob(Knob::HashFair) ? c->d_counts.p + 7 : nullptr,
+                                    (uint32_t)knob(Knob::HashFairEvery)));
+    HIP_OK(c, hipEventRecord(c->pfx_ev[1], ps));
+    c->have_prefix = true;
+  }
   HIP_OK(c, hipEventRecord(c->ev[1], st));
   HIP_OK(c, hipEventRecord(c->ev[2], st));
   if (nfiles)
@@ -654,19 +700,21 @@
                             (uint64_t)p.max_chunk, c->d_slots.p, c->d_nseg.p,
                             c->d_unit_ctr.p + 2, c->d_segs.p, c->d_seg_begin.p, c->d_order.p,
                             c->d_qctr.p, st, bin_bytes, bin_bytes ? c->d_next.p : nullptr,
-                            c->d_counts.p + 4));
+                            c->d_counts.p + 4, pfx_bytes));
   const uint64_t* qlen = c->d_counts.p + 4;
   const uint32_t* next = bin_bytes ? c->d_next.p : nullptr;
   HIP_OK(c, hipEventRecord(c->ev[3], st));
   if (c->hash_after && c->hash_after->device == c->device)
     HIP_OK(c, hipStreamWaitEvent(st, c->hash_after->ev[4], 0));
+  if (prefix) HIP_OK(c, hipStreamWaitEvent(st, c->pfx_ev[1], 0));
   if (nfiles && !(options & kScanNoHash))
     HIP_OK(c, launch_blake2b(data, c->d_offs.p, c->d_segs.p, qlen, cap,
                              c->d_order.p, c->d_qctr.p, c->num_cus, nbytes, st, true,
                              c->d_span.p + 2, waves, 0u, waves == 1, next,
                              knob(Knob::HashFair) && waves > 1 && next ? c->d_counts.p + 5
                                                                       : nullptr,
-                             (uint32_t)knob(Knob::HashFairEvery)));
+                             (uint32_t)knob(Knob::HashFairEvery), prefix ? c->d_mid.p : nullptr,
+                             (uint64_t)p.min_chunk));
   HIP_OK(c, hipEventRecord(c->ev[4], st));
   c->have_refs = (options & PFSCDC_OPT_REF_IDS) != 0 && !(options & kScanNoHash);
   if (c->have_refs && nfiles)
@@ -696,7 +744,8 @@
   const uint32_t o = c->options;
   const bool cuts = (o & PFSCDC_OPT_CUTS_ONLY) != 0;
   const int rc = scan_async_impl(c, bytes, nbytes, bytes_on_device, file_offsets, nfiles,
-                                 (o & ~PFSCDC_OPT_CUTS_ONLY) | (cuts ? kScanNoHash : 0u));
+                                 (o & ~PFSCDC_OPT_CUTS_ONLY) | (cuts ? kScanNoHash : 0u) |
+                                     kScanPrefix);
   if (rc == PFSCDC_OK) c->cuts_only = cuts;
   return rc;
 }
@@ -873,6 +922,17 @@
   PFS_HIP(c, hipEventElapsedTime(&out[2], c->ev[2], c->ev[3]));
   PFS_HIP(c, hipEventElapsedTime(&out[3], c->ev[3], c->ev[4]));
   PFS_HIP(c, hipEventElapsedTime(&out[4], c->ev[0], c->ev[4]));
+  return PFSCDC_OK;
+}
+
+int pfscdc_last_prefix_timings(pfscdc_ctx* c, float out[2]) {
+  if (!c || !out) return PFSCDC_EINVAL;
+  if (c->pending) return fail(c, PFSCDC_ESTATE, "scan pending");
+  out[0] = out[1] = 0.f;
+  if (!c->have_prefix || !c->h_span.p) return PFSCDC_OK;
+  PFS_HIP(c, hipEventElapsedTime(&out[0], c->pfx_ev[0], c->pfx_ev[1]));
+  const uint64_t a = c->h_span.p[8], b = c->h_span.p[9];
+  if (b > a && a != ~0ULL) out[1] = (float)((double)(b - a) / c->wall_khz);
   return PFSCDC_OK;
 }
 
diff --git a/pfs_amd/csrc/pfscdc_internal.h b/pfs_amd/csrc/pfscdc_internal.h
--- a/pfs_amd/csrc/pfscdc_internal.h
+++ b/pfs_amd/csrc/pfscdc_internal.h
@@ -39,7 +39,7 @@
 
 enum class Knob : int {
   ScanSkip, ScanCutSkip, ScanGrid, HashGrid, ChachaGrid,
-  HashBinBytes, HashWaves, HashFair, HashFairEvery,
+  HashBinBytes, HashWaves, HashFair, HashFairEvery, HashPrefix,
   RefIdSplit, CommitTwoSets, CommitLongPct,
   UwWorkers, UwInflight, UwMirror, UwIndexGrouped, UwArenaPoolBytes, CtxCache, CopyThreads,
   IndexDecode, IndexMerge, Source, Diff, CopyMap, Trace,
@@ -58,6 +58,7 @@
 void go_int63(int64_t seed, int64_t* out, int n);
 
 constexpr uint32_t kScanNoHash = 0x100;
+constexpr uint32_t kScanPrefix = 0x200;
 int hash_records_device(pfscdc_ctx* ctx, const uint8_t* data, uint64_t nbytes,
                         const uint64_t* begins, const uint64_t* sizes, uint32_t n, uint8_t* out);
 int scan_sync(pfscdc_ctx* ctx, const void* bytes, uint64_t nbytes, int bytes_on_device,
@@ -122,7 +123,8 @@
                          uint64_t* nseg, uint32_t* done_ctr, pfscdc_segment* segs,
                          uint64_t* seg_begin, uint32_t* order, uint32_t* counter,
                          hipStream_t st, uint64_t bin_bytes = 0, uint32_t* next = nullptr,
-                         uint64_t* qlen = nullptr);
+                         uint64_t* qlen = nullptr,
+                         uint64_t pfx_bytes = 0);
 constexpr uint32_t kHashPrioAuto = 0x3fffffffu;
 constexpr uint32_t kHashPrioNone = 0x80000000u;
 hipError_t launch_blake2b(const uint8_t* data, const uint64_t* offs, pfscdc_segment* segs,
@@ -133,7 +135,15 @@
                           bool cu_exclusive = false,
                           const uint32_t* next = nullptr,
                           uint64_t* fair = nullptr,
-                          uint32_t fair_every = 256);
+                          uint32_t fair_every = 256,
+                          const uint64_t* mid = nullptr,
+                          uint64_t pfx_min = 0);
+constexpr uint32_t kMidStateWords = 9;
+hipError_t launch_blake2b_prefix(const uint8_t* data, const uint64_t* offs, uint32_t nfiles,
+                                 uint64_t nprefix, uint64_t pfx_min, uint32_t pfx_blocks,
+                                 uint64_t* mid, uint32_t* counter, int num_cus, uint64_t nbytes,
+                                 hipStream_t st, uint64_t* span, int waves, uint64_t* fair,
+                                 uint32_t fair_every);
 int hash_waves(uint64_t longest_bytes, uint64_t total_bytes, int num_cus, int forced);
 hipError_t launch_order(const pfscdc_segment* segs, const uint64_t* seg_count, uint32_t* order,
                         uint32_t* counter, hipStream_t st);
```
